# chao1224/GeoSSL

Measured on AMD Instinct MI355X. Metric: molecules/s/GPU SchNet+DDM fwd+bwd (QM9-sized, bs=1024); % HBM roofline, higher is better.
Workload: dtype f32

## Files before the change

geossl_amd/NCSN.py:

```python
import ctypes as C
import os

import numpy as np
import torch
from .switches import env as _env
import torch.nn as nn
import torch.nn.functional as F

from . import _lib
from ._lib import call, ptr, stream
from .layout import get_super_edge_layout


class MultiLayerPerceptron(nn.Module):

    def __init__(self, input_dim, hidden_dims, activation="relu", dropout=0):
        super().__init__()
        self.dims = [input_dim] + hidden_dims
        self.activation = getattr(F, activation) if isinstance(activation, str) else None
        self.dropout = nn.Dropout(dropout) if dropout else None
        self.layers = nn.ModuleList()
        for i in range(len(self.dims) - 1):
            self.layers.append(nn.Linear(self.dims[i], self.dims[i + 1]))
        self.reset_parameters()

    def reset_parameters(self):
        for layer in self.layers:
            nn.init.xavier_uniform_(layer.weight)
            nn.init.constant_(layer.bias, 0.0)

    def forward(self, input):
        from .higher_order import _linear_wide
        _lib.require_cuda(input)
        lead = input.shape[:-1]
        x = input.reshape(-1, input.shape[-1])
        for i, layer in enumerate(self.layers):
            x = _linear_wide(x, layer.weight, layer.bias)
            if i < len(self.layers) - 1:
                if self.activation:
                    x = self.activation(x)
                if self.dropout:
                    x = self.dropout(x)
        return x.reshape(*lead, x.shape[-1])


def _head_params(m):
    i, o = m.input_distance_mlp.layers, m.output_mlp.layers
    return [i[0].weight, i[0].bias, i[1].weight, i[1].bias, o[0].weight, o[0].bias, o[1].weight, o[1].bias,
            o[2].weight, o[2].bias]


_FIELDS = ("in_w1", "in_b1", "in_w2", "in_b2", "o1_w", "o1_b", "o2_w", "o2_b", "o3_w", "o3_b")

_SIDE = {"stream": None, "pending": []}


def set_side_stream(stream):
    _SIDE["stream"] = stream


def join_side_stream():
    if _SIDE["pending"]:
        for ev, _keep in _SIDE["pending"]:
            torch.cuda.current_stream().wait_event(ev)
        _SIDE["pending"].clear()


class _NcsnLoss(torch.autograd.Function):
    @staticmethod
    def forward(ctx, h, distance, noise_level, distance_noise, sel, sigmas, anneal_power, out_scale, *params):
        dev = h.device
        S, Fd = sel.S, h.size(1)
        training = ctx.needs_input_grad[0] or any(ctx.needs_input_grad[8:])
        ps = [p.detach().contiguous() for p in params]
        w = _lib.NcsnWeights()
        for name, p in zip(_FIELDS, ps):
            setattr(w, name, ptr(p))
        w.sigmas = ptr(sigmas)
        ctx.grad_slot = getattr(h, "_geossl_grad_slot", None)
        h = h.detach().contiguous()
        loss_e = torch.empty(S, dtype=torch.float32, device=dev)
        sv = None
        saved = {}
        if training:
            saved = dict(a1=torch.empty(S, Fd, dtype=torch.float32, device=dev),
                         a2=torch.empty(S, Fd // 2, dtype=torch.float32, device=dev),
                         pd=torch.empty(S, dtype=torch.float32, device=dev),
                         emb=torch.empty(S, dtype=torch.float32, device=dev),
                         gscale=torch.empty(S, dtype=torch.float32, device=dev))
            sv = _lib.NcsnSaved(*[ptr(saved[k]) for k in ("a1", "a2", "pd", "emb", "gscale")])
        lib = _lib.load()
        nws = max(int(lib.geossl_ddm_loss_fwd_workspace_floats(Fd)), 256)
        ws = (torch.empty if S > 0 else torch.zeros)(nws, dtype=torch.float32, device=dev)
        st = stream()
        call("geossl_ddm_loss_fwd", ptr(h), ptr(sel.batch), ptr(sel.sei0), ptr(sel.sei1), S,
             ptr(distance.contiguous()), ptr(noise_level.contiguous()), ptr(distance_noise.contiguous()), C.byref(w),
             Fd, float(anneal_power), ptr(loss_e), C.byref(sv) if sv is not None else None, ptr(ws), st)
        loss = torch.empty((), dtype=torch.float32, device=dev)
        call("geossl_loss_reduce_partials", ptr(ws), ptr(sel.stats), float(out_scale), ptr(loss), 0, st)
        if training:
            ctx.sel, ctx.ps, ctx.w, ctx.saved, ctx.h = sel, ps, w, saved, h
            ctx.params = params
            ctx.sigmas = sigmas
            ctx.out_scale = float(out_scale)
        return loss

    @staticmethod
    def backward(ctx, gout):
        sel, ps, w, saved, h = ctx.sel, ctx.ps, ctx.w, ctx.saved, ctx.h
        dev = h.device
        S, Fd, N = sel.S, h.size(1), h.size(0)
        st = stream()
        sv = _lib.NcsnSaved(*[ptr(saved[k]) for k in ("a1", "a2", "pd", "emb", "gscale")])
        dfeat = torch.empty(S, Fd, dtype=torch.float32, device=dev)
        demb = torch.empty(S, dtype=torch.float32, device=dev)
        grow = torch.empty(S, dtype=torch.float32, device=dev)
        gout = gout.contiguous().to(torch.float32)
        direct = _lib.direct_grads_enabled(ctx.params)
        grads = [p.grad for p in ctx.params] if direct else [torch.empty_like(p) for p in ps]
        g = _lib.NcsnGrads(*[ptr(t) for t in grads])
        lib = _lib.load()
        acc = 1 if direct else 0
        split = (_env("GEOSSL_NCSN_SPLIT_BWD") is not None or _env("GEOSSL_ARITH_24BIT") is not None
                 or max(S, N) * Fd * 4 >= 2 ** 32)
        if not split:
            ws1 = torch.empty(int(lib.geossl_ddm_loss_bwd_fused_workspace_floats(S, Fd)), dtype=torch.float32, device=dev)
            call("geossl_ddm_loss_bwd_fused", ptr(h), ptr(sel.sei0), ptr(sel.sei1), S, N, Fd, C.byref(w), C.byref(sv),
                 ptr(sel.stats), ctx.out_scale, ptr(gout), ptr(dfeat), ptr(demb), ptr(grow), C.byref(g), ptr(ws1), acc, st)
            dz1 = None
        else:
            dz1 = torch.empty(S, Fd, dtype=torch.float32, device=dev)
            call("geossl_ddm_loss_bwd_rows", C.byref(w), C.byref(sv), S, Fd, ptr(sel.stats), ctx.out_scale, ptr(gout),
                 ptr(dz1), ptr(dfeat), ptr(demb), ptr(grow), st)
        dh = None
        if ctx.needs_input_grad[0]:
            slot = ctx.grad_slot
            dh = slot.rows(N, Fd, torch.float32, dev) if slot is not None else None
            if dh is None:
                dh = torch.empty(N, Fd, dtype=torch.float32, device=dev)
            call("geossl_incidence_gather", ptr(dfeat), ptr(sel.inc_ptr), ptr(sel.inc_idx), N, Fd, ptr(dh), 0, st)
        if split:
            nfl = lib.geossl_ddm_loss_bwd_workspace_floats(S, Fd)
            side = _SIDE["stream"] if direct else None
            if side is None:
                ws = torch.empty(nfl, dtype=torch.float32, device=dev)
                call("geossl_ddm_loss_bwd_weights", ptr(h), ptr(sel.sei0), ptr(sel.sei1), S, Fd, C.byref(w), C.byref(sv),
                     ptr(dz1), ptr(demb), ptr(grow), C.byref(g), ptr(ws), acc, st)
            else:
                main = torch.cuda.current_stream()
                fork = torch.cuda.Event()
                fork.record(main)
                side.wait_event(fork)
                with torch.cuda.stream(side):
                    ws = torch.empty(nfl, dtype=torch.float32, device=dev)
                    call("geossl_ddm_loss_bwd_weights", ptr(h), ptr(sel.sei0), ptr(sel.sei1), S, Fd, C.byref(w),
                         C.byref(sv), ptr(dz1), ptr(demb), ptr(grow), C.byref(g), ptr(ws), 1, stream())
                    done = torch.cuda.Event()
                    done.record(side)
                _SIDE["pending"].append((done, (h, saved, dz1, demb, grow, ws, w, sv, ps, grads)))
        if direct:
            return (dh, None, None, None, None, None, None, None) + (None,) * len(grads)
        return (dh, None, None, None, None, None, None, None) + tuple(grads)


class _NcsnLossPair(torch.autograd.Function):

    @staticmethod
    def forward(ctx, h1, h2, d1, d2, nl1, dn1, nl2, dn2, sel, sigmas, powers, out_scale, npar, *params):
        dev = h1.device
        S, Fd, N = sel.S, h1.size(1), h1.size(0)
        training = ctx.needs_input_grad[0] or ctx.needs_input_grad[1] or any(ctx.needs_input_grad[13:])
        ps = [p.detach().contiguous() for p in params]
        pss = (ps[:npar], ps[npar:])
        dyn = getattr(sel, "dyn", None)
        ctx.dyn = dyn
        if dyn is not None:
            hs = (h1.detach().contiguous(),) * 2
            ctx.grad_slots = (None, None)
        else:
            hs = (h1.detach().contiguous(), h2.detach().contiguous())
            ctx.grad_slots = (getattr(h1, "_geossl_grad_slot", None), getattr(h2, "_geossl_grad_slot", None))
        heads = (_lib.NcsnHeadFwd * 2)()
        keep, saved, ws = [], [], []
        for k, (h, d, nl, dn) in enumerate(((hs[0], d1, nl1, dn1), (hs[1], d2, nl2, dn2))):
            hd = heads[k]
            d, nl, dn = d.contiguous(), nl.contiguous(), dn.contiguous()
            keep += [d, nl, dn]
            for name, p in zip(_FIELDS, pss[k]):
                setattr(hd.w, name, ptr(p))
            hd.w.sigmas = ptr(sigmas[k])
            hd.h, hd.distance, hd.noise_level, hd.distance_noise = ptr(h), ptr(d), ptr(nl), ptr(dn)
            hd.anneal_power = float(powers[k])
            loss_e = torch.empty(S, dtype=torch.float32, device=dev)
            sv = {}
            if training:
                sv = dict(a1=torch.empty(S, Fd, dtype=torch.float32, device=dev),
                          a2=torch.empty(S, Fd // 2, dtype=torch.float32, device=dev),
                          pd=torch.empty(S, dtype=torch.float32, device=dev),
                          emb=torch.empty(S, dtype=torch.float32, device=dev),
                          gscale=torch.empty(S, dtype=torch.float32, device=dev))
                for name in ("a1", "a2", "pd", "emb", "gscale"):
                    setattr(hd.saved, name, ptr(sv[name]))
            w_ = torch.empty(256, dtype=torch.float32, device=dev)
            hd.loss_e, hd.workspace = ptr(loss_e), ptr(w_)
            keep.append(loss_e)
            saved.append(sv)
            ws.append(w_)
        st = stream()
        call("geossl_ddm_loss_fwd2_dyn", C.byref(heads), ptr(sel.batch), ptr(sel.sei0), ptr(sel.sei1), S, Fd,
             None if dyn is None else dyn.n_super, None if dyn is None else dyn.n_atoms, st)
        loss = torch.empty((), dtype=torch.float32, device=dev)
        call("geossl_loss_reduce_partials2", ptr(ws[0]), ptr(ws[1]), ptr(sel.stats), float(out_scale), float(out_scale),
             ptr(loss), st)
        if training:
            ctx.sel, ctx.pss, ctx.saved, ctx.hs, ctx.sigmas = sel, pss, saved, hs, sigmas
            ctx.params, ctx.npar, ctx.out_scale = params, npar, float(out_scale)
        return loss

    @staticmethod
    def backward(ctx, gout):
        sel, pss, saved, hs = ctx.sel, ctx.pss, ctx.saved, ctx.hs
        dev = hs[0].device
        S, Fd, N = sel.S, hs[0].size(1), hs[0].size(0)
        st = stream()
        gout = gout.contiguous().to(torch.float32)
        direct = _lib.direct_grads_enabled(ctx.params)
        grads = [p.grad for p in ctx.params] if direct else [torch.empty_like(p) for p in pss[0] + pss[1]]
        gs = (grads[:ctx.npar], grads[ctx.npar:])
        lib = _lib.load()
        heads = (_lib.NcsnHeadBwd * 2)()
        keep, dhs = [], []
        nws = int(lib.geossl_ddm_loss_bwd_fused_workspace_floats(S, Fd))
        dyn = ctx.dyn
        dh_all = torch.empty(N, Fd, dtype=torch.float32, device=dev) if dyn is not None else None
        for k in range(2):
            hd = heads[k]
            for name, p in zip(_FIELDS, pss[k]):
                setattr(hd.w, name, ptr(p))
            hd.w.sigmas = ptr(ctx.sigmas[k])
            for name in ("a1", "a2", "pd", "emb", "gscale"):
                setattr(hd.saved, name, ptr(saved[k][name]))
            for name, t_ in zip(_FIELDS, gs[k]):
                setattr(hd.grads, name, ptr(t_))
            dfeat = torch.empty(S, Fd, dtype=torch.float32, device=dev)
            demb = torch.empty(S, dtype=torch.float32, device=dev)
            grow = torch.empty(S, dtype=torch.float32, device=dev)
            ws1 = torch.empty(nws, dtype=torch.float32, device=dev)
            slot = ctx.grad_slots[k]
            dh = dh_all if dyn is not None else (slot.rows(N, Fd, torch.float32, dev) if slot is not None else None)
            if dh is None:
                dh = torch.empty(N, Fd, dtype=torch.float32, device=dev)
            hd.h, hd.out_scale, hd.dfeat, hd.demb, hd.grow, hd.workspace, hd.dh = (
                ptr(hs[k]), ctx.out_scale, ptr(dfeat), ptr(demb), ptr(grow), ptr(ws1), ptr(dh))
            keep += [dfeat, demb, grow, ws1]
            dhs.append(dh)
        call("geossl_ddm_loss_bwd_fused2_dyn", C.byref(heads), ptr(sel.sei0), ptr(sel.sei1), S, sel.N if dyn is not None else N,
             Fd, ptr(sel.stats), ptr(gout), ptr(sel.inc_ptr), ptr(sel.inc_idx), 1 if direct else 0,
             None if dyn is None else dyn.n_super, None if dyn is None else dyn.n_atoms, st)
        head = ((dh_all, None) if dyn is not None else (dhs[0], dhs[1])) + (None,) * 11
        if direct:
            return head + (None,) * len(grads)
        return head + tuple(grads)


def ddm_heads_loss(n1, n2, data, h1, distance_1, h2, distance_2, noise_level_1=None, distance_noise_1=None,
                   noise_level_2=None, distance_noise_2=None, out_scale=0.5):
    ok = (isinstance(n1, NCSN_version_03) and isinstance(n2, NCSN_version_03) and n1.emb_dim == n2.emb_dim
          and n1.emb_dim in (32, 64, 128) and not _env("GEOSSL_NCSN_SPLIT_BWD")
          and not _env("GEOSSL_ARITH_24BIT")
          and not _env("GEOSSL_NCSN_SEPARATE_HEADS")
          and (h2 is None or h1.shape == h2.shape) and not distance_1.requires_grad and not distance_2.requires_grad
          and n1 is not n2 and not ({id(p) for p in _head_params(n1)} & {id(p) for p in _head_params(n2)}))
    if ok:
        S_, N_, Fd = data.super_edge_index.size(1), h1.size(0), h1.size(1)
        ok = S_ > 0 and max(S_, N_) * Fd * 4 < 2 ** 32
    bucket = getattr(data, "_bucket", None)
    if bucket is not None and (not ok or h2 is not None):
        raise _lib.GeosslHipError("a capacity-bucket batch needs the paired NCSN heads on one fused feature tensor")
    if not ok:
        return (n1(data, h1, distance_1, noise_level=noise_level_1, distance_noise=distance_noise_1, out_scale=out_scale) +
                n2(data, h2, distance_2, noise_level=noise_level_2, distance_noise=distance_noise_2, out_scale=out_scale))
    _lib.require_cuda(h1, h2, distance_1, distance_2, n1.sigmas, n2.sigmas)
    n1.device = n2.device = n1.sigmas.device
    num_graphs = data.num_graphs
    sel = bucket.sel if bucket is not None else get_super_edge_layout(data.batch, data.super_edge_index, num_graphs)
    draws = []
    for n_, nl, dn, d in ((n1, noise_level_1, distance_noise_1, distance_1), (n2, noise_level_2, distance_noise_2, distance_2)):
        if nl is None:
            nl = torch.randint(0, n_.sigmas.size(0), (num_graphs,), device=n_.sigmas.device)
        if dn is None:
            dn = torch.randn_like(d)
        draws.append((nl, dn))
    p1, p2 = _head_params(n1), _head_params(n2)
    return _NcsnLossPair.apply(h1, h2, distance_1.view(-1), distance_2.view(-1), draws[0][0], draws[0][1].view(-1),
                               draws[1][0], draws[1][1].view(-1), sel, (n1.sigmas.detach(), n2.sigmas.detach()),
                               (n1.anneal_power, n2.anneal_power), out_scale, len(p1), *p1, *p2)


class NCSN_version_03(torch.nn.Module):
    def __init__(self, emb_dim, sigma_begin, sigma_end, num_noise_level, noise_type, anneal_power):
        super().__init__()
        self.anneal_power = anneal_power
        self.noise_type = noise_type
        self.input_distance_mlp = MultiLayerPerceptron(1, [emb_dim, 1], activation="relu")
        self.output_mlp = MultiLayerPerceptron(1 + emb_dim, [emb_dim, emb_dim // 2, 1])
        sigmas = torch.tensor(np.exp(np.linspace(np.log(sigma_begin), np.log(sigma_end), num_noise_level)),
                              dtype=torch.float32)
        self.sigmas = nn.Parameter(sigmas, requires_grad=False)
        self.emb_dim = emb_dim

    def forward(self, data, node_feature, distance, debug=False, noise_level=None, distance_noise=None,
                out_scale=1.0):
        self.device = self.sigmas.device
        _lib.require_cuda(node_feature, distance, self.sigmas)
        if self.emb_dim not in (32, 64, 128):
            raise NotImplementedError("HIP path supports emb_dim in (32, 64, 128)")
        if distance.requires_grad:
            raise NotImplementedError("gradient w.r.t. distance/positions is not built (SURVEY.md §8(f) N3)")
        num_graphs = data.num_graphs
        sel = get_super_edge_layout(data.batch, data.super_edge_index, num_graphs)
        if noise_level is None:
            noise_level = torch.randint(0, self.sigmas.size(0), (num_graphs,), device=self.device)
        if distance_noise is None:
            distance_noise = torch.randn_like(distance)
        if sel.S == 0:
            raise ValueError("batch has no super edges (scatter_add over an empty index fails in the reference too)")
        loss = _NcsnLoss.apply(node_feature, distance.view(-1), noise_level, distance_noise.view(-1), sel,
                               self.sigmas.detach(), self.anneal_power, out_scale, *_head_params(self))
        if debug:
            print("loss", float(loss))
        return loss
```

geossl_amd/_lib.py:

```python
import ctypes as C
import os

import torch

HERE = os.path.dirname(os.path.abspath(__file__))
LIB_PATH = os.path.join(HERE, "lib", "libgeossl_hip.so")

MAX_L = 12
TN_MAX = 32
EPI_BIAS, EPI_SSP, EPI_RESIDUAL, EPI_MUL_DSSP, CHAIN_SAME_INPUT, CHAIN_NEW_INPUT, CHAIN_ADD_PREV = 1, 2, 4, 8, 16, 32, 64
EPI_SILU, EPI_MUL_DSILU = 128, 256

vp = C.c_void_p
i64 = C.c_int64
i32 = C.c_int
f32 = C.c_float
f64 = C.c_double
u64 = C.c_uint64


class FilterWeights(C.Structure):
    _fields_ = [("w1", vp * MAX_L), ("b1", vp * MAX_L), ("w2", vp * MAX_L), ("b2", vp * MAX_L)]


PREPARE_MAX = 64


class PrepareBatch(C.Structure):
    _fields_ = [("W", vp * PREPARE_MAX), ("image", vp * PREPARE_MAX), ("ldw", i32 * PREPARE_MAX), ("tb", i32 * PREPARE_MAX)]


CHAIN_MAX = 5


class ChainStage(C.Structure):
    _fields_ = [("image", vp), ("bias", vp), ("res", vp), ("tprev", vp), ("out", vp), ("ld", i32), ("flags", i32),
                ("xin", vp), ("ldxin", i32), ("pad_", i32), ("out_act", vp)]


class Chain(C.Structure):
    _fields_ = [("nstage", i32), ("st", ChainStage * CHAIN_MAX)]


LOOP_MAX_OPS = 14


class LoopOp(C.Structure):
    _fields_ = [("kind", i32), ("swap", i32), ("X", vp), ("Wf", vp), ("out", vp), ("chain", Chain)]


class FilterGradIn(C.Structure):
    _fields_ = [("x", vp * MAX_L), ("dagg", vp * MAX_L)]


class FilterGradOut(C.Structure):
    _fields_ = [("dw1", vp * MAX_L), ("db1", vp * MAX_L), ("dw2", vp * MAX_L), ("db2", vp * MAX_L)]


class TnBatch(C.Structure):
    _fields_ = [("A", vp * TN_MAX), ("B", vp * TN_MAX), ("dW", vp * TN_MAX), ("db", vp * TN_MAX)]


class NcsnWeights(C.Structure):
    _fields_ = [(k, vp) for k in ("in_w1", "in_b1", "in_w2", "in_b2", "o1_w", "o1_b", "o2_w", "o2_b", "o3_w", "o3_b",
                                  "sigmas")]


class NcsnGrads(C.Structure):
    _fields_ = [(k, vp) for k in ("in_w1", "in_b1", "in_w2", "in_b2", "o1_w", "o1_b", "o2_w", "o2_b", "o3_w", "o3_b")]


class NcsnSaved(C.Structure):
    _fields_ = [(k, vp) for k in ("a1", "a2", "pd", "emb", "gscale")]


class NcsnHeadFwd(C.Structure):
    _fields_ = [("h", vp), ("distance", vp), ("noise_level", vp), ("distance_noise", vp), ("w", NcsnWeights),
                ("saved", NcsnSaved), ("anneal_power", f32), ("pad_", f32), ("loss_e", vp), ("workspace", vp)]


class NcsnHeadBwd(C.Structure):
    _fields_ = [("h", vp), ("w", NcsnWeights), ("saved", NcsnSaved), ("out_scale", f32), ("pad_", f32), ("dfeat", vp),
                ("demb", vp), ("grow", vp), ("grads", NcsnGrads), ("workspace", vp), ("dh", vp)]


COPY_MAX = 8


class CopyBatch(C.Structure):
    _fields_ = [("dst", vp * COPY_MAX), ("src", vp * COPY_MAX), ("bytes", i64 * COPY_MAX)]


class Gather(C.Structure):
    _fields_ = [(k, vp) for k in ("x_src", "pos_src", "src_off", "mol_ptr", "x_dst", "pos_dst", "batch_dst", "se_ptr", "sei0",
                                  "sei1", "pair_ptr2", "pair_i", "pair_j", "inc_ptr", "inc_idx", "e0_src", "e1_src",
                                  "e_src_off", "e_ptr", "e0_dst", "e1_dst", "zero")] + \
               [("zero_count", i64), ("x_cols", i32), ("option", i32)]


P = C.POINTER
PROTOTYPES = {
    "geossl_abi_version": (i32, []),
    "geossl_layout_build": (i32, [vp, i64, i64, vp, vp, vp, vp]),
    "geossl_pair_index_fill": (i32, [vp, vp, i64, vp, vp, vp]),
    "geossl_radius_graph_count": (i32, [vp, vp, i64, i32, f32, i32, vp, vp]),
    "geossl_radius_graph_fill": (i32, [vp, vp, i64, i32, f32, i32, vp, vp, vp, vp, vp]),
    "geossl_pair_geometry": (i32, [vp, vp, vp, i64, i32, f32, i32, f32, vp, vp, vp, vp]),
    "geossl_rbf_fwd": (i32, [vp, i64, vp, i32, f32, vp, vp]),
    "geossl_ssp_fwd": (i32, [vp, i64, vp, vp]),
    "geossl_ssp_bwd": (i32, [vp, vp, i64, vp, vp]),
    "geossl_cfconv_filter_fwd": (i32, [vp, vp, i64, P(FilterWeights), i32, i32, i32, vp, f32, vp, vp, vp]),
    "geossl_cfconv_filter_bwd_workspace_floats": (i64, [i64, i32, i32, i32]),
    "geossl_cfconv_filter_bwd": (i32, [vp, vp, vp, vp, vp, i64, i64, P(FilterWeights), P(FilterGradIn), i32, i32, i32, vp,
                                       f32, vp, P(FilterGradOut), vp, i32, vp]),
    "geossl_cfconv_filter_dpos": (i32, [vp, vp, vp, vp, vp, i64, P(FilterWeights), P(FilterGradIn), i32, i32, i32, vp, f32,
                                        f32, vp, vp, vp, vp]),
    "geossl_pair_position_grad": (i32, [vp, vp, vp, vp, vp, i64, i64, i32, vp, vp]),
    "geossl_cfconv_aggregate": (i32, [vp, vp, vp, vp, vp, vp, i64, i32, i32, i32, vp, vp]),
    "geossl_aggregate_parts": (i32, [i32]),
    "geossl_cfconv_aggregate_work": (i32, [vp, vp, vp, vp, vp, vp, i64, i32, i32, i32, vp, vp]),
    "geossl_pair_product": (i32, [vp, vp, vp, vp, vp, i64, i32, i32, vp, vp]),
    "geossl_linear": (i32, [vp, i32, vp, vp, vp, vp, vp, i32, i64, i32, i32, i32, i32, vp]),
    "geossl_tn_plan": (None, [i64, i32, P(i32), P(i32)]),
    "geossl_tn_workspace_floats": (i64, [i64, i32, i32, i32]),
    "geossl_row_normalize_fwd": (i32, [vp, i64, i32, f32, vp, vp, vp]),
    "geossl_row_normalize_bwd": (i32, [vp, vp, vp, i64, i32, f32, vp, vp]),
    "geossl_atom_tuples": (i32, [vp, vp, i64, i32, vp, vp, vp]),
    "geossl_linear_image_words": (i64, [i32, i32]),
    "geossl_linear_prepare": (i32, [P(PrepareBatch), i32, i32, i32, i32, vp]),
    "geossl_linear_prepared": (i32, [vp, i32, vp, vp, vp, vp, vp, i32, i64, i32, i32, i32, vp]),
    "geossl_chain_image_words": (i64, [i32]),
    "geossl_chain_prepare": (i32, [P(PrepareBatch), i32, i32, i32, vp]),
    "geossl_linear_chain": (i32, [vp, i32, P(Chain), i64, i32, vp]),
    "geossl_linear_wgrad": (i32, [P(TnBatch), i32, i64, i32, i32, i32, i32, i32, vp, i32, vp]),
    "geossl_embedding_fwd": (i32, [vp, i64, vp, i32, i64, i32, vp, vp, vp]),
    "geossl_embedding_bwd_workspace_floats": (i64, [i32, i32]),
    "geossl_embedding_bwd": (i32, [vp, i64, vp, i32, i64, i32, vp, vp, i32, vp]),
    "geossl_segment_reduce_fwd": (i32, [vp, vp, i64, i32, i32, vp, vp]),
    "geossl_segment_reduce_bwd": (i32, [vp, vp, i64, i32, i32, vp, i32, vp]),
    "geossl_axpy": (i32, [vp, vp, f32, i64, vp, vp]),
    "geossl_pair_distance": (i32, [vp, vp, vp, i64, vp, vp]),
    "geossl_super_edge_ptr": (i32, [vp, vp, vp, i64, i64, vp, vp, vp]),
    "geossl_incidence_count": (i32, [vp, vp, vp, vp, i64, i32, vp, vp]),
    "geossl_incidence_fill": (i32, [vp, vp, vp, vp, i64, i32, vp, vp, vp]),
    "geossl_ddm_loss_fwd_workspace_floats": (i64, [i32]),
    "geossl_ddm_loss_fwd": (i32, [vp, vp, vp, vp, i64, vp, vp, vp, P(NcsnWeights), i32, f32, vp, P(NcsnSaved), vp, vp]),
    "geossl_schnet_layer_loop": (i32, [vp, i32, vp, i32, vp, vp, vp, i32, i32, i64, i32, i32, vp]),
    "geossl_schnet_layer_loop_ragged": (i32, [vp, i32, vp, vp, vp, i64, i32, i64, i32, vp]),
    "geossl_copy2": (i32, [vp, vp, i64, vp, vp, i64, vp]),
    "geossl_ddm_noise": (i32, [vp, f32, f32, i64, i64, i64, i32, i32, vp, vp, vp, vp, vp, vp]),
    "geossl_ddm_noise_seeded": (i32, [u64, f32, f32, i64, i64, i64, i32, i32, vp, vp, vp, vp, vp, vp]),
    "geossl_ddm_views": (i32, [vp, vp, vp, vp, i64, i64, vp, vp, vp, vp, i64, vp, vp]),
    "geossl_loss_reduce_partials": (i32, [vp, vp, f32, vp, i32, vp]),
    "geossl_ddm_loss_fwd2": (i32, [vp, vp, vp, vp, i64, i32, vp]),
    "geossl_loss_reduce_partials2": (i32, [vp, vp, vp, f32, f32, vp, vp]),
    "geossl_ddm_loss_bwd_fused2": (i32, [vp, vp, vp, i64, i64, i32, vp, vp, vp, vp, i32, vp]),
    "geossl_loss_reduce_workspace_floats": (i64, [i64]),
    "geossl_loss_reduce": (i32, [vp, i64, vp, f32, vp, vp, i32, vp]),
    "geossl_ddm_loss_bwd_rows": (i32, [P(NcsnWeights), P(NcsnSaved), i64, i32, vp, f32, vp, vp, vp, vp, vp, vp]),
    "geossl_ddm_loss_bwd_workspace_floats": (i64, [i64, i32]),
    "geossl_ddm_loss_bwd_weights": (i32, [vp, vp, vp, i64, i32, P(NcsnWeights), P(NcsnSaved), vp, vp, vp, P(NcsnGrads),
                                          vp, i32, vp]),
    "geossl_ddm_loss_bwd_fused_workspace_floats": (i64, [i64, i32]),
    "geossl_ddm_loss_bwd_fused": (i32, [vp, vp, vp, i64, i64, i32, P(NcsnWeights), P(NcsnSaved), vp, f32, vp, vp, vp, vp,
                                        P(NcsnGrads), vp, i32, vp]),
    "geossl_incidence_gather": (i32, [vp, vp, vp, i64, i32, vp, i32, vp]),
    "geossl_painn_edge_geom": (i32, [vp, vp, vp, i64, f32, vp, vp, i32, vp, vp, vp, vp]),
    "geossl_silu_fwd": (i32, [vp, i64, vp, vp]),
    "geossl_silu_bwd": (i32, [vp, vp, i64, vp, vp]),
    "geossl_painn_interaction_fwd": (i32, [vp, vp, vp, vp, vp, vp, vp, vp, vp, vp, vp, i64, i32, i32, vp, vp, vp]),
    "geossl_painn_interaction_bwd_workspace_floats": (i64, [i64, i32, i32]),
    "geossl_painn_interaction_fwd_mol": (i32, [vp, vp, vp, vp, vp, vp, vp, vp, vp, vp, vp, vp, i64, i32, i64, i32, i32, vp,
                                               vp, vp]),
    "geossl_painn_interaction_fwd_mma": (i32, [vp, vp, vp, vp, vp, vp, vp, vp, vp, vp, vp, vp, vp, i64, i32, i64, i32, i32,
                                               vp, vp, vp]),
    "geossl_painn_interaction_bwd_mol_workspace_floats": (i64, [i64, i64, i32, i32]),
    "geossl_painn_interaction_bwd_mol": (i32, [vp, vp, vp, vp, vp, vp, vp, vp, vp, vp, vp, vp, vp, i64, i32, i64, i32, i32,
                                               vp, vp, vp, vp, vp, i32, vp]),
    "geossl_painn_interaction_bwd": (i32, [vp, vp, vp, vp, vp, vp, vp, vp, vp, vp, vp, vp, i64, i32, i32, vp, vp, vp, vp,
                                           vp, i32, vp]),
    "geossl_painn_mix_pre_fwd": (i32, [vp, vp, i64, i32, f32, vp, vp, vp]),
    "geossl_painn_mix_post_fwd": (i32, [vp, vp, vp, vp, vp, i64, i32, vp, vp, vp]),
    "geossl_painn_mix_post_bwd": (i32, [vp, vp, vp, vp, vp, i64, i32, vp, vp, vp]),
    "geossl_painn_mix_pre_bwd": (i32, [vp, vp, vp, vp, i64, i32, vp, vp, vp]),
    "geossl_add": (i32, [vp, vp, i64, vp, vp]),
    "geossl_painn_edge_grads": (i32, [vp] * 11 + [i64, i32, i32, vp, vp, vp, i32, vp]),
    "geossl_painn_edge_geom_bwd": (i32, [vp, vp, vp, i64, f32, vp, vp, i32, vp, vp, vp, vp, vp]),
    "geossl_painn_position_grad": (i32, [vp, vp, vp, vp, vp, i64, vp, vp]),
    "geossl_adam_step": (i32, [vp, vp, vp, vp, i64, f64, f64, f64, f64, f64, i64, f32, vp]),
    "geossl_copy_n": (i32, [P(CopyBatch), i32, vp]),
    "geossl_ddm_views_dyn": (i32, [vp, vp, vp, vp, i64, i64, vp, vp, vp, vp, i64, vp, vp, vp, vp]),
    "geossl_embedding_fwd_dyn": (i32, [vp, i64, vp, i32, i64, i32, vp, vp, vp, vp]),
    "geossl_embedding_bwd_dyn": (i32, [vp, i64, vp, i32, i64, i32, vp, vp, i32, vp, vp]),
    "geossl_cfconv_filter_fwd_dyn": (i32, [vp, vp, i64, P(FilterWeights), i32, i32, i32, vp, f32, vp, vp, vp, vp]),
    "geossl_cfconv_filter_bwd_dyn": (i32, [vp, vp, vp, vp, vp, i64, i64, P(FilterWeights), P(FilterGradIn), i32, i32, i32,
                                           vp, f32, vp, P(FilterGradOut), vp, i32, vp, vp, vp]),
    "geossl_cfconv_aggregate_work_dyn": (i32, [vp, vp, vp, vp, vp, vp, i64, i32, i32, i32, vp, vp, vp]),
    "geossl_cfconv_aggregate_targets_dyn": (i32, [vp, vp, vp, vp, vp, vp, i64, i32, i32, i32, vp, vp, vp]),
    "geossl_linear_chain_dyn": (i32, [vp, i32, P(Chain), i64, i32, vp, vp]),
    "geossl_linear_wgrad_dyn": (i32, [P(TnBatch), i32, i64, i32, i32, i32, i32, i32, vp, i32, vp, vp]),
    "geossl_ddm_loss_fwd2_dyn": (i32, [vp, vp, vp, vp, i64, i32, vp, vp, vp]),
    "geossl_ddm_loss_bwd_fused2_dyn": (i32, [vp, vp, vp, i64, i64, i32, vp, vp, vp, vp, i32, vp, vp, vp]),
    "geossl_painn_group_capacity": (i64, [i64, i64]),
    "geossl_painn_edge_layout": (i32, [vp, vp, i64, vp, i64, i64, i64] + [vp] * 12),
    "geossl_painn_edge_geom_dyn": (i32, [vp, vp, vp, i64, f32, vp, vp, i32, vp, vp, vp, vp, vp]),
    "geossl_painn_interaction_fwd_mma_dyn": (i32, [vp, vp, vp, vp, vp, vp, vp, vp, vp, vp, vp, vp, vp, i64, i32, i64, i32,
                                                   i32, vp, vp, vp, vp]),
    "geossl_tape_unary": (i32, [i32, vp, i64, f32, f32, vp, vp]),
    "geossl_tape_binary": (i32, [i32, vp, i32, vp, i32, i64, i32, f32, vp, vp]),
    "geossl_tape_colsum_workspace_floats": (i64, [i64, i32]),
    "geossl_tape_reduce": (i32, [i32, vp, i64, i32, vp, vp, vp]),
    "geossl_tape_gather_rows": (i32, [vp, vp, i32, i64, i32, vp, vp]),
    "geossl_tape_scatter_rows": (i32, [vp, vp, i32, vp, i64, i32, vp, vp]),
    "geossl_tape_copy2d": (i32, [vp, i64, vp, i64, i64, i32, vp]),
    "geossl_tape_fill": (i32, [vp, i64, f32, vp]),
    "geossl_painn_stage_cap": (i32, [i32, i32, i32]),
    "geossl_painn_interaction_fwd_atoms": (i32, [vp] * 12 + [i64, vp, i32, i32, vp, vp, vp]),
    "geossl_painn_interaction_bwd_atoms": (i32, [vp] * 13 + [i64, vp, i32, i32, vp, vp, vp, vp, vp, i32, vp]),
    "geossl_painn_interaction_bwd_mol_skip": (i32, [vp, vp, vp, vp, vp, vp, vp, vp, vp, vp, vp, vp, vp, i64, i32, i64, i32,
                                                    i32, vp, vp, vp, vp, vp, i32, vp]),
    "geossl_painn_mix_pre_fwd_dyn": (i32, [vp, vp, i64, i32, f32, vp, vp, vp, vp]),
    "geossl_painn_mix_post_fwd_dyn": (i32, [vp, vp, vp, vp, vp, i64, i32, vp, vp, vp, vp]),
    "geossl_painn_mix_post_bwd_dyn": (i32, [vp, vp, vp, vp, vp, i64, i32, vp, vp, vp, vp]),
    "geossl_painn_mix_pre_bwd_dyn": (i32, [vp, vp, vp, vp, i64, i32, vp, vp, vp, vp]),
    "geossl_gather_molecules": (i32, [P(Gather), i64, vp]),
}

_lib = None


class GeosslHipError(RuntimeError):
    pass


def load():
    global _lib
    if _lib is not None:
        return _lib
    path = os.environ.get("GEOSSL_HIP_LIB", LIB_PATH)
    if not os.path.exists(path):
        raise GeosslHipError(
            "libgeossl_hip.so is not built (%s). Run `python -m geossl_amd.build` (needs hipcc); "
            "there is no CPU fallback." % path)
    lib = C.CDLL(path)
    for name, (res, args) in PROTOTYPES.items():
        fn = getattr(lib, name)
        fn.restype = res
        fn.argtypes = args
    if lib.geossl_abi_version() != 1:
        raise GeosslHipError("ABI version mismatch")
    _lib = lib
    return lib


def check(rc, what):
    if rc != 0:
        raise GeosslHipError("%s failed with hipError %d" % (what, rc))


def ptr(t):
    if t is None:
        return None
    return t.data_ptr()


def stream():
    return torch._C._cuda_getCurrentRawStream(torch._C._cuda_getDevice())


def require_cuda(*tensors):
    for t in tensors:
        if t is not None and not t.is_cuda:
            raise GeosslHipError(
                "geossl_amd runs on MI355X only: got a %s tensor. The HIP path has no CPU fallback." % t.device.type)



_DIRECT = {"depth": 0}


class direct_grads:
    def __enter__(self):
        _DIRECT["depth"] += 1
        return self

    def __exit__(self, *exc):
        _DIRECT["depth"] -= 1
        return False


def direct_grads_enabled(params):
    return _DIRECT["depth"] > 0 and all(
        p.grad is not None and p.grad.is_contiguous() and p.grad.dtype == torch.float32 and p.grad.is_cuda
        for p in params)


class StatusWord:

    def __init__(self, device, message):
        self.word = torch.zeros(1, dtype=torch.int32, device=device)
        self.host = torch.zeros(1, dtype=torch.int32).pin_memory()
        self.event = None
        self.message = message

    def __deepcopy__(self, memo):
        return None

    def __reduce__(self):
        return (type(None), ())

    def poll(self):
        if self.event is None or torch.cuda.is_current_stream_capturing():
            return
        if self.event.query():
            self.event = None
            if int(self.host[0]):
                raise IndexError(self.message)

    def arm(self, every=1):
        self.calls = getattr(self, "calls", 0) + 1
        if every > 1 and self.calls % every != 1:
            return
        if self.event is None and not torch.cuda.is_current_stream_capturing():
            self.host.copy_(self.word, non_blocking=True)
            self.event = torch.cuda.Event()
            self.event.record()

    def check(self):
        if int(self.word.item()):
            raise IndexError(self.message)


def module_status(module, device, message):
    st = module.__dict__.get("_geossl_status")
    if st is None or st.word.device != device:
        st = StatusWord(device, message)
        module.__dict__["_geossl_status"] = st
    return st


TIMERS = None
CALLS = None


def call(name, *args):
    global CALLS
    lib = load()
    if CALLS is not None:
        CALLS += 1
    timers = TIMERS
    key = name[:-4] if name.endswith("_dyn") else name
    if timers is not None and key in timers:
        e0, e1 = torch.cuda.Event(enable_timing=True), torch.cuda.Event(enable_timing=True)
        e0.record()
        rc = getattr(lib, name)(*args)
        e1.record()
        timers[key].append((e0, e1))
    else:
        rc = getattr(lib, name)(*args)
    check(rc, name)


def fill_ptrs(arr, tensors):
    for i, t in enumerate(tensors):
        arr[i] = ptr(t)
```

geossl_amd/csrc/common.h:

```cpp
#pragma once
#include <hip/hip_runtime.h>
#include <stdint.h>

#include <mutex>

typedef float f32x16 __attribute__((ext_vector_type(16)));
typedef float f32x4 __attribute__((ext_vector_type(4)));

#define GEOSSL_MAX_LAYERS 12
#define GEOSSL_PI_F 3.14159265358979323846f

#define GEOSSL_CHECK_LAUNCH()                  \
  do {                                         \
    hipError_t e__ = hipGetLastError();        \
    if (e__ != hipSuccess) return (int)e__;    \
  } while (0)

namespace geossl {

inline void allow_big_lds_ptr(const void* kernel) {
  struct Seen { const void* fn; int dev; };
  static Seen seen[512];
  static int nseen = 0;
  static std::mutex mu;
  int dev = 0;
  if (hipGetDevice(&dev) != hipSuccess) dev = -1;
  std::lock_guard<std::mutex> lock(mu);
  for (int i = 0; i < nseen; ++i)
    if (seen[i].fn == kernel && seen[i].dev == dev) return;
  (void)hipFuncSetAttribute(kernel, hipFuncAttributeMaxDynamicSharedMemorySize, 160 * 1024);
  if (dev >= 0 && nseen < 512) seen[nseen++] = Seen{kernel, dev};
}
template <typename K>
inline void allow_big_lds(K kernel) { allow_big_lds_ptr(reinterpret_cast<const void*>(kernel)); }


__device__ __forceinline__ float mul_rn(float a, float b) {
#pragma clang fp contract(off)
  return a * b;
}
__device__ __forceinline__ float add_rn(float a, float b) {
#pragma clang fp contract(off)
  return a + b;
}
__device__ __forceinline__ float norm2_rn(float x, float y, float z) {
#pragma clang fp contract(off)
  const float xx = x * x, yy = y * y, zz = z * z;
  return (xx + yy) + zz;
}

__device__ __forceinline__ void lds_barrier() {
  asm volatile("s_waitcnt lgkmcnt(0)\n\ts_barrier" ::: "memory");
}

__device__ __forceinline__ float wave_max(float v) {
  v = fmaxf(v, __builtin_bit_cast(float, __builtin_amdgcn_update_dpp(0, __builtin_bit_cast(int, v), 0xB1, 0xF, 0xF, false)));
  v = fmaxf(v, __builtin_bit_cast(float, __builtin_amdgcn_update_dpp(0, __builtin_bit_cast(int, v), 0x4E, 0xF, 0xF, false)));
  v = fmaxf(v, __builtin_bit_cast(float, __builtin_amdgcn_update_dpp(0, __builtin_bit_cast(int, v), 0x141, 0xF, 0xF, false)));
  v = fmaxf(v, __builtin_bit_cast(float, __builtin_amdgcn_update_dpp(0, __builtin_bit_cast(int, v), 0x140, 0xF, 0xF, false)));
  const float a = __builtin_bit_cast(float, __builtin_amdgcn_readlane(__builtin_bit_cast(int, v), 0));
  const float b = __builtin_bit_cast(float, __builtin_amdgcn_readlane(__builtin_bit_cast(int, v), 16));
  const float c = __builtin_bit_cast(float, __builtin_amdgcn_readlane(__builtin_bit_cast(int, v), 32));
  const float d = __builtin_bit_cast(float, __builtin_amdgcn_readlane(__builtin_bit_cast(int, v), 48));
  return fmaxf(fmaxf(a, b), fmaxf(c, d));
}
__device__ __forceinline__ int wave_max_i32(int v) {
  v = max(v, __builtin_amdgcn_update_dpp(v, v, 0xB1, 0xF, 0xF, false));
  v = max(v, __builtin_amdgcn_update_dpp(v, v, 0x4E, 0xF, 0xF, false));
  v = max(v, __builtin_amdgcn_update_dpp(v, v, 0x141, 0xF, 0xF, false));
  v = max(v, __builtin_amdgcn_update_dpp(v, v, 0x140, 0xF, 0xF, false));
  return max(max(__builtin_amdgcn_readlane(v, 0), __builtin_amdgcn_readlane(v, 16)),
             max(__builtin_amdgcn_readlane(v, 32), __builtin_amdgcn_readlane(v, 48)));
}
__device__ __forceinline__ int c_row(int reg, int lane) { return (reg & 3) + 8 * (reg >> 2) + 4 * (lane >> 5); }

#define GEOSSL_SSP_SHIFT 0.693147182464599609375f
__device__ __forceinline__ float exp_neg(float x) { return __builtin_amdgcn_exp2f(x * 1.44269504088896340736f); }
__device__ __forceinline__ float ssp(float x) {
  const float z = exp_neg(-fabsf(x));
  const float l = __builtin_amdgcn_logf(1.0f + z);
  return fmaf(l, 0.693147180559945309417f, fmaxf(x, 0.0f)) - GEOSSL_SSP_SHIFT;
}
__device__ __forceinline__ float dssp_from_out(float t) { return 1.0f - 0.5f * exp_neg(-t); }

template <class ValFn, class ConsumeFn>
__device__ __forceinline__ void transpose_c_block(float* stage, int lane, ValFn val, ConsumeFn consume) {
  const int j = lane & 31, kh = lane >> 5;
  const int rr = lane >> 3, c4 = lane & 7;
#pragma unroll
  for (int half = 0; half < 2; ++half) {
#pragma unroll
    for (int q = 0; q < 8; ++q) {
      const int r = 8 * half + q;
      const int row16 = (r & 3) + 8 * ((r >> 2) & 1) + 4 * kh;
      stage[row16 * 32 + j] = val(r);
    }
    asm volatile("s_waitcnt lgkmcnt(0)" ::: "memory");
#pragma unroll
    for (int u = 0; u < 2; ++u) {
      const int row16 = 8 * u + rr;
      const float4 v = *reinterpret_cast<const float4*>(stage + row16 * 32 + 4 * c4);
      consume(16 * half + row16, 4 * c4, v);
    }
    asm volatile("s_waitcnt lgkmcnt(0)" ::: "memory");
  }
}

__device__ __forceinline__ float pin(float v) {
  asm volatile("" : "+v"(v));
  return v;
}
__device__ __forceinline__ float4 pin(float4 v) {
  asm volatile("" : "+v"(v.x), "+v"(v.y), "+v"(v.z), "+v"(v.w));
  return v;
}

__device__ __forceinline__ float kahan_sum_strided(const float* __restrict__ p, int b0, int b1, int stride) {
#pragma clang fp reassociate(off) contract(off)
  float s = 0.0f, c = 0.0f;
#pragma unroll 4
  for (int b = b0; b < b1; ++b) {
    const float y = p[(size_t)b * stride] - c;
    const float t = s + y;
    c = (t - s) - y;
    s = t;
  }
  return s;
}

__device__ __forceinline__ int dyn_count(int cap, const int32_t* __restrict__ dyn) {
  return dyn != nullptr ? min(cap, *dyn) : cap;
}

__device__ __forceinline__ float wave_sum(float v) {
#pragma unroll
  for (int o = 32; o > 0; o >>= 1) v += __shfl_xor(v, o, 64);
  return v;
}

}
```

geossl_amd/csrc/ncsn_bwd.hip:

```cpp
#include "common.h"
#include "geossl_hip.h"
#include "split.h"
#include "tn.h"

using namespace geossl;

namespace {

constexpr int TR = 32;

#ifdef NB_TIMING
__device__ long long nb_dbg[2 * 32 * 8];
#define NB_MARK(slot)                                                                              \
  do {                                                                                             \
    if (blockIdx.x == 5 && lane == 0 && (wave == 0 || wave == NW) && t - t_begin < 32)             \
      nb_dbg[((wave == 0 ? 0 : 1) * 32 + (t - t_begin)) * 8 + (slot)] = clock64();                 \
  } while (0)
#else
#define NB_MARK(slot) do {} while (0)
#endif

template <int NW>
struct NbLds {
  static constexpr int F = 32 * NW, H = F / 2, KHS = (H + 15) / 16, HMB = (H + 31) / 32, KS = F / 16;
  u32x4* zb;
  u32x4* dz2T;
  u32x4* fT;
  u32x4* dz1r;
  u32x4* abT;
  int4* scal;
  float* pdv;
  float* dep;
  float* wls;
  int* eg;
  int* ef;
  int* ea;
  int* ec;
  __device__ explicit NbLds(uint8_t* smem) {
    zb = reinterpret_cast<u32x4*>(smem);
    dz2T = zb + 2 * KHS * 2 * 64;
    fT = dz2T + HMB * 2 * 2 * 64;
    dz1r = fT + 2 * NW * 2 * 2 * 64;
    abT = dz1r + KS * 2 * 64;
    scal = reinterpret_cast<int4*>(abT + NW * 2 * 2 * 64);
    pdv = reinterpret_cast<float*>(scal + 3 * TR);
    dep = pdv + 3 * TR;
    wls = dep + NW * TR;
    eg = reinterpret_cast<int*>(wls + F);
    ef = eg + 4;
    ea = ef + 2 * NW;
    ec = ea + NW;
  }
  static size_t bytes() {
    return (size_t)(2 * KHS * 2 + HMB * 4 + 2 * NW * 4 + KS * 2 + NW * 4) * 1024 + 3 * TR * sizeof(int4) +
           (size_t)(3 * TR + NW * TR + F) * sizeof(float) + (size_t)(4 + 4 * NW) * sizeof(int);
  }
};

struct NcsnFusedArgs {
  const float* h;
  const int64_t* sei0;
  const int64_t* sei1;
  int S;
  GeosslNcsnWeights w;
  GeosslNcsnSaved sv;
  const int64_t* divisor;
  float out_scale;
  const float* gout;
  float* dfeat;
  float* demb;
  float* grow;
  float* pw1;
  float* pd1;
  float* pb1;
  float* pw2;
  float* pb2;
  float* psm;
};

__device__ __forceinline__ float ldg_off(const float* base, uint32_t byte_off) {
  return *reinterpret_cast<const float*>(reinterpret_cast<const char*>(base) + byte_off);
}
__device__ __forceinline__ int crow4(int r, int k4) { return (r & 3) + 8 * (r >> 2) + k4; }
__device__ __forceinline__ int opaque(int v) {
  asm volatile("" : "+v"(v));
  return v;
}
__device__ __forceinline__ u32x4 pack8(const f32x16& t, int s) {
  u32x4 w;
#pragma unroll
  for (int q = 0; q < 4; ++q) {
    const f16x2 p = {(_Float16)t[8 * s + 2 * q], (_Float16)t[8 * s + 2 * q + 1]};
    w[q] = __builtin_bit_cast(uint32_t, p);
  }
  return w;
}
__device__ __forceinline__ const u32x4& piece(const Frag2& f, int pc) { return pc == 0 ? f.h : f.l; }
__device__ __forceinline__ int scale_exponent(float m) { return max(mag_exponent(m), -40); }
__device__ __forceinline__ float pow2(int e) { return __builtin_amdgcn_ldexpf(1.0f, e); }
constexpr int E_NONE = -100000;

template <int NW, bool ROLE_A>
__device__ __forceinline__ void ncsn_bwd_body(const NcsnFusedArgs& a, const int S, const float* __restrict__ a_h) {
  using L_t = NbLds<NW>;
  constexpr int F = L_t::F, H = L_t::H, KHS = L_t::KHS, HMB = L_t::HMB, KS = L_t::KS, NT = 128 * NW;
  extern __shared__ __attribute__((aligned(16))) uint8_t smem_raw[];
  const L_t L(smem_raw);
  const int tid = threadIdx.x, lane = tid & 63, j = lane & 31, kh = lane >> 5;
  const int wave = __builtin_amdgcn_readfirstlane(tid >> 6);
  const int nb = ROLE_A ? wave : wave - NW;
  const int ntiles = (S + TR - 1) / TR;
  const int per = (ntiles + (int)gridDim.x - 1) / (int)gridDim.x;
  const int t_begin = (int)blockIdx.x * per, t_end = min(ntiles, t_begin + per);
  const float scale = a.out_scale * (a.gout != nullptr ? a.gout[0] : 1.0f) / (float)a.divisor[0];
  const uint32_t col = 32 * nb + j;

  Frag2 wreg[ROLE_A ? KHS : KS];
  f32x16 accw1[ROLE_A ? NW : 1];
  f32x16 accw2[ROLE_A ? 1 : HMB];
  int E1[ROLE_A ? NW : 1];
  int E2 = E_NONE;
  int ew = 0;
  float bsum = 0.0f, dsum = 0.0f;
  u32x4 ident[2];
  float w3r[8];
  float s_w2 = 0.0f, s_w1 = 0.0f, s_b1 = 0.0f, s_g = 0.0f, s_d = 0.0f;
  float iw1 = 0.0f, ib1 = 0.0f, iw2 = 0.0f;
  int e3;
  {
    float m3 = 0.0f;
    for (int i = lane; i < H; i += 64) m3 = fmaxf(m3, fabsf(a.w.o3_w[i]));
    e3 = scale_exponent(wave_max(m3));
  }
  if constexpr (ROLE_A) {
    iw1 = a.w.in_w1[col];
    ib1 = a.w.in_b1[col];
    iw2 = a.w.in_w2[col];
    float raw[KHS][8];
    float wm = 0.0f, csum = 0.0f;
#pragma unroll
    for (int ks = 0; ks < KHS; ++ks)
#pragma unroll
      for (int e = 0; e < 8; ++e) {
        const int m = 16 * ks + 8 * kh + e;
        const float v = m < H ? a.w.o2_w[(size_t)m * F + col] : 0.0f;
        raw[ks][e] = v;
        wm = fmaxf(wm, fabsf(v));
        csum = fmaf(fabsf(v), m < H ? fabsf(a.w.o3_w[m]) : 0.0f, csum);
      }
    ew = scale_exponent(wave_max(wm));
    const float sw = pow2(14 - ew);
#pragma unroll
    for (int ks = 0; ks < KHS; ++ks) wreg[ks] = split8h_scaled(raw[ks], sw);
    csum += __shfl_xor(csum, 32, 64);
    const int ecw = max(mag_exponent(wave_max(csum)), -80);
    if (lane == 0) L.ec[nb] = ecw;
#pragma unroll
    for (int kb = 0; kb < NW; ++kb) {
      E1[kb] = E_NONE;
#pragma unroll
      for (int r = 0; r < 16; ++r) accw1[kb][r] = 0.0f;
    }
#pragma unroll
    for (int s = 0; s < 2; ++s)
#pragma unroll
      for (int q = 0; q < 4; ++q) {
        const int k0 = 16 * s + kperm(2 * q, kh), k1 = 16 * s + kperm(2 * q + 1, kh);
        ident[s][q] = (k0 == j ? 0x3C00u : 0u) | (k1 == j ? 0x3C000000u : 0u);
      }
  } else {
    float raw[KS][8];
    float wm = 0.0f;
#pragma unroll
    for (int ks = 0; ks < KS; ++ks)
#pragma unroll
      for (int e = 0; e < 8; ++e) {
        raw[ks][e] = a.w.o1_w[(size_t)(16 * ks + kperm(e, kh)) * (F + 1) + col];
        wm = fmaxf(wm, fabsf(raw[ks][e]));
      }
    ew = scale_exponent(wave_max(wm));
    const float sw = pow2(14 - ew);
#pragma unroll
    for (int ks = 0; ks < KS; ++ks) wreg[ks] = split8h_scaled(raw[ks], sw);
#pragma unroll
    for (int e = 0; e < 8; ++e) {
      const int m = 16 * nb + 8 * kh + e;
      w3r[e] = (nb < KHS && m < H) ? a.w.o3_w[m] : 0.0f;
    }
#pragma unroll
    for (int mb = 0; mb < HMB; ++mb)
#pragma unroll
      for (int r = 0; r < 16; ++r) accw2[mb][r] = 0.0f;
#pragma unroll
    for (int q2 = 0; q2 < 2; ++q2)
#pragma unroll
      for (int q = 0; q < 4; ++q) {
        const int k0 = 16 * q2 + 8 * kh + 2 * q;
        ident[q2][q] = (k0 == j ? 0x3C00u : 0u) | (k0 + 1 == j ? 0x3C000000u : 0u);
      }
  }
  for (int i = tid; i < F; i += NT) L.wls[i] = a.w.o1_w[(size_t)i * (F + 1) + F];

  int sc_u = 0, sc_v = 0;
  float sc_g = 0.0f, sc_e = 0.0f, sc_p = 0.0f;
  int EG = -60;
  auto load_scal = [&](int tt) {
    if constexpr (ROLE_A) {
      if (wave == 0) {
        const int row = min(TR * tt + j, S - 1);
        sc_u = (int)a.sei0[row];
        sc_v = (int)a.sei1[row];
        sc_g = a.sv.gscale[row];
        sc_e = a.sv.emb[row];
        sc_p = a.sv.pd[row];
      }
    }
  };
  auto put_scal = [&](int tt) {
    if constexpr (ROLE_A) {
      if (wave == 0) {
        const int row = TR * tt + lane;
        const bool valid = lane < TR && row < S && tt < t_end;
        const float gr = valid ? pin(sc_g) * scale : 0.0f;
        EG = max(EG, mag_exponent(wave_max(fabsf(gr))));
        if (lane < TR) {
          L.scal[(tt % 3) * TR + lane] = make_int4(sc_u, sc_v, __float_as_int(gr), __float_as_int(sc_e));
          L.pdv[(tt % 3) * TR + lane] = sc_p;
          if (valid) a.grow[row] = gr;
        }
        if (lane == 0) L.eg[tt % 3] = EG;
      }
    }
  };
  float a1raw[16];
  auto request_a1 = [&](int tt, int k4) {
    if constexpr (ROLE_A) {
#pragma unroll
      for (int r = 0; r < 16; ++r)
        a1raw[r] = ldg_off(a.sv.a1, ((uint32_t)min(TR * tt + crow4(r, k4), S - 1) * (uint32_t)F + col) * 4u);
    }
  };
  f32x4 a2raw[2];
  float o3acc[8] = {0.0f, 0.0f, 0.0f, 0.0f, 0.0f, 0.0f, 0.0f, 0.0f};
  auto request_a2 = [&](int tt) {
    if constexpr (!ROLE_A) {
      if (nb < KHS) {
        const uint32_t off = ((uint32_t)min(TR * tt + j, S - 1) * (uint32_t)H + (16 * nb + 8 * kh)) * 4u;
        a2raw[0] = *reinterpret_cast<const f32x4*>(reinterpret_cast<const char*>(a.sv.a2) + off);
        a2raw[1] = *reinterpret_cast<const f32x4*>(reinterpret_cast<const char*>(a.sv.a2) + 16 + off);
      }
    }
  };
  float hu[16], hv[16];
  auto request_gather = [&](int tt, int k4) {
    if constexpr (!ROLE_A) {
      const int2* sc = reinterpret_cast<const int2*>(L.scal + (tt % 3) * TR);
#pragma unroll
      for (int r = 0; r < 16; ++r) {
        const int2 uv = sc[2 * crow4(r, k4)];
        hu[r] = ldg_off(a_h, ((uint32_t)uv.x * (uint32_t)F + col) * 4u);
        hv[r] = ldg_off(a_h, ((uint32_t)uv.y * (uint32_t)F + col) * 4u);
      }
    }
  };
  auto build_zb = [&](int tt) {
    if constexpr (!ROLE_A) {
      if (nb < KHS) {
        const float gr = __int_as_float(L.scal[(tt % 3) * TR + j].z);
        const float sz = pow2(14 - e3 - __builtin_amdgcn_readfirstlane(L.eg[tt % 3]));
        const float av[8] = {a2raw[0].x, a2raw[0].y, a2raw[0].z, a2raw[0].w, a2raw[1].x, a2raw[1].y, a2raw[1].z, a2raw[1].w};
        float v[8];
#pragma unroll
        for (int e = 0; e < 8; ++e) {
          const float a2v = pin(av[e]);
          v[e] = a2v > 0.0f ? gr * w3r[e] : 0.0f;
          o3acc[e] = fmaf(gr, a2v, o3acc[e]);
        }
        const Frag2 f = split8h_scaled(v, sz);
        u32x4* dst = L.zb + (size_t)(((tt & 1) * KHS + nb) * 2) * 64 + lane;
        dst[0] = f.h;
        dst[64] = f.l;
      }
    }
  };
  int EF = -40;
  auto build_fT = [&](int tt) {
    if constexpr (!ROLE_A) {
      float v[16];
      float m = 0.0f;
#pragma unroll
      for (int r = 0; r < 16; ++r) {
        v[r] = pin(hu[r]) + pin(hv[r]);
        m = fmaxf(m, fabsf(v[r]));
      }
      EF = max(EF, mag_exponent(wave_max(m)));
      const float sf = pow2(14 - EF);
      if (lane == 0) L.ef[(tt & 1) * NW + nb] = EF;
#pragma unroll
      for (int s = 0; s < 2; ++s) {
        float vv[8];
#pragma unroll
        for (int e = 0; e < 8; ++e) vv[e] = v[8 * s + e];
        const Frag2 f = split8h_scaled(vv, sf);
        u32x4* dst = L.fT + (size_t)((((tt & 1) * NW + nb) * 2 + s) * 2) * 64 + lane;
        dst[0] = f.h;
        dst[64] = f.l;
      }
    }
  };

  load_scal(t_begin);
  put_scal(t_begin);
  load_scal(t_begin + 1);
  put_scal(t_begin + 1);
  load_scal(t_begin + 2);
  if (t_begin < t_end) {
    request_a1(t_begin, 4 * kh);
    request_a2(t_begin);
  }
  __syncthreads();
  int eC = -80;
#pragma unroll
  for (int i = 0; i < NW; ++i) eC = max(eC, __builtin_amdgcn_readfirstlane(L.ec[i]));
  if (t_begin < t_end) {
    request_gather(t_begin, 4 * kh);
    build_zb(t_begin);
    build_fT(t_begin);
    request_a2(t_begin + 1);
    request_gather(t_begin + 1, 4 * kh);
  }
  int EA = -40;
  const float kA = pow2(e3 + ew - eC - 14);
  for (int t = t_begin; t < t_end; ++t) {
    const int buf = t & 1;
    int k4 = opaque(4 * kh);
    NB_MARK(0);
    lds_barrier();
    NB_MARK(1);
    const int EGt = __builtin_amdgcn_readfirstlane(L.eg[t % 3]);
    if constexpr (ROLE_A) {
      put_scal(t + 2);
      const float kT = pow2(EGt + eC - 14);
      f32x16 acc0, acc1;
#pragma unroll
      for (int r = 0; r < 16; ++r) acc0[r] = acc1[r] = 0.0f;
      {
        const u32x4* zs = L.zb + (size_t)(buf * KHS * 2) * 64 + lane;
        Frag2 a0, an;
        a0.h = zs[0]; a0.l = zs[64];
#pragma unroll
        for (int ks = 0; ks < KHS; ++ks) {
          if (ks + 1 < KHS) {
            const u32x4* s0 = zs + (size_t)((ks + 1) * 2) * 64;
            an.h = s0[0]; an.l = s0[64];
          }
          __builtin_amdgcn_sched_barrier(0);
          mma3x2(acc0, acc1, a0, wreg[ks]);
          __builtin_amdgcn_sched_barrier(0);
          if (ks + 1 < KHS) a0 = an;
        }
      }
      NB_MARK(5);
      float v[16];
      {
        const int4* sc = L.scal + (t % 3) * TR;
        float tb = 0.0f, td = 0.0f, am = 0.0f;
#pragma unroll
        for (int r = 0; r < 16; ++r) {
          a1raw[r] = pin(a1raw[r]);
          v[r] = a1raw[r] > 0.0f ? (acc0[r] + acc1[r]) * kA : 0.0f;
          tb += v[r];
          td = fmaf(v[r], __int_as_float(sc[crow4(r, k4)].w), td);
          am = fmaxf(am, fabsf(a1raw[r]));
        }
        bsum = fmaf(tb, kT, bsum);
        dsum = fmaf(td, kT, dsum);
        EA = max(EA, mag_exponent(wave_max(am)));
      }
      {
        const float sa = pow2(14 - EA);
        if (lane == 0) L.ea[nb] = EA;
#pragma unroll
        for (int s = 0; s < 2; ++s) {
          float vv[8];
#pragma unroll
          for (int e = 0; e < 8; ++e) vv[e] = a1raw[8 * s + e];
          const Frag2 f = split8h_scaled(vv, sa);
          u32x4* dst = L.abT + (size_t)((nb * 2 + s) * 2) * 64 + lane;
          dst[0] = f.h;
          dst[64] = f.l;
        }
      }
      Frag2 da[2];
#pragma unroll
      for (int s = 0; s < 2; ++s) {
        float vv[8];
#pragma unroll
        for (int e = 0; e < 8; ++e) vv[e] = v[8 * s + e];
        da[s] = split8h(vv);
      }
      {
        float wl[16];
#pragma unroll
        for (int r = 0; r < 16; ++r) wl[r] = L.wls[32 * nb + crow4(r, k4)];
        float de = 0.0f;
#pragma unroll
        for (int pc = 1; pc >= 0; --pc) {
          f32x16 tp;
#pragma unroll
          for (int r = 0; r < 16; ++r) tp[r] = 0.0f;
          tp = mfma_f16(piece(da[0], pc), ident[0], tp);
          tp = mfma_f16(piece(da[1], pc), ident[1], tp);
#pragma unroll
          for (int r = 0; r < 16; ++r) de = fmaf(tp[r], wl[r], de);
#pragma unroll
          for (int half = 0; half < 2; ++half)
            L.dz1r[(size_t)((2 * nb + half) * 2 + pc) * 64 + lane] = pack8(tp, half);
        }
        de += __shfl_xor(de, 32, 64);
        if (kh == 0) L.dep[j * NW + nb] = de * kT;
      }
      NB_MARK(6);
#pragma unroll
      for (int kb = 0; kb < NW; ++kb) {
        const int En = EGt + __builtin_amdgcn_readfirstlane(L.ef[buf * NW + kb]);
        if (En != E1[kb]) {
          const float f = pow2(max(E1[kb] - En, -200));
#pragma unroll
          for (int r = 0; r < 16; ++r) accw1[kb][r] *= f;
          E1[kb] = En;
        }
#pragma unroll
        for (int s = 0; s < 2; ++s) {
          const u32x4* s0 = L.fT + (size_t)(((buf * NW + kb) * 2 + s) * 2) * 64 + lane;
          Frag2 bf;
          bf.h = s0[0]; bf.l = s0[64];
          mma3(accw1[kb], da[s], bf);
        }
      }
    } else {
      if (nb < HMB) {
        float tb = 0.0f;
#pragma unroll
        for (int pc = 1; pc >= 0; --pc) {
          f32x16 tp;
#pragma unroll
          for (int r = 0; r < 16; ++r) tp[r] = 0.0f;
#pragma unroll
          for (int q = 0; q < 2; ++q) {
            if (2 * nb + q < KHS) {
              const u32x4* s0 = L.zb + (size_t)((buf * KHS + 2 * nb + q) * 2 + pc) * 64 + lane;
              tp = mfma_f16(s0[0], ident[q], tp);
            }
          }
#pragma unroll
          for (int r = 0; r < 16; ++r) tb += tp[r];
#pragma unroll
          for (int s = 0; s < 2; ++s) L.dz2T[(size_t)((nb * 2 + s) * 2 + pc) * 64 + lane] = pack8(tp, s);
        }
        bsum = fmaf(tb, pow2(EGt + e3 - 14), bsum);
      }
      NB_MARK(5);
      build_zb(t + 1);
      NB_MARK(6);
      build_fT(t + 1);
    }
    k4 = opaque(4 * kh);
    NB_MARK(2);
    lds_barrier();
    NB_MARK(3);
    if constexpr (ROLE_A) {
      request_a1(t + 1, k4);
      load_scal(t + 3);
      {
        const int4* sc = L.scal + (t % 3) * TR;
        const float* pdr = L.pdv + (t % 3) * TR;
#pragma unroll
        for (int i = 0; i < 16; ++i) {
          const int rl = 4 * k4 + i;
          float de = 0.0f;
#pragma unroll
          for (int n2 = 0; n2 < NW; ++n2) de += L.dep[rl * NW + n2];
          const float pd = pdr[rl];
          const float pre = fmaf(iw1, pd, ib1);
          s_w2 = fmaf(de, fmaxf(pre, 0.0f), s_w2);
          const float dp = pre > 0.0f ? de * iw2 : 0.0f;
          s_w1 = fmaf(dp, pd, s_w1);
          s_b1 += dp;
          if (wave == 0 && j == i) {
            s_g += __int_as_float(sc[rl].z);
            s_d += de;
          }
        }
      }
    } else {
      request_a2(t + 2);
      request_gather(t + 2, k4);
      NB_MARK(7);
      f32x16 acc0, acc1;
#pragma unroll
      for (int r = 0; r < 16; ++r) acc0[r] = acc1[r] = 0.0f;
      {
        const u32x4* zs = L.dz1r + lane;
        Frag2 b0, bn;
        b0.h = zs[0]; b0.l = zs[64];
#pragma unroll
        for (int ks = 0; ks < KS; ++ks) {
          if (ks + 1 < KS) {
            const u32x4* s0 = zs + (size_t)((ks + 1) * 2) * 64;
            bn.h = s0[0]; bn.l = s0[64];
          }
          __builtin_amdgcn_sched_barrier(0);
          mma3x2(acc0, acc1, wreg[ks], b0);
          __builtin_amdgcn_sched_barrier(0);
          if (ks + 1 < KS) b0 = bn;
        }
      }
      const float kD = pow2(EGt + eC + ew - 28);
      f32x16 outp;
#pragma unroll
      for (int r = 0; r < 16; ++r) outp[r] = (acc0[r] + acc1[r]) * kD;
      const int row = TR * t + j;
      if (row < S) {
        const uint32_t off = ((uint32_t)row * (uint32_t)F + 32 * nb + 4 * kh) * 4u;
#pragma unroll
        for (int q = 0; q < 4; ++q)
          *reinterpret_cast<f32x4*>(reinterpret_cast<char*>(a.dfeat) + 32 * q + off) =
              f32x4{outp[4 * q], outp[4 * q + 1], outp[4 * q + 2], outp[4 * q + 3]};
        if (nb == 0 && kh == 0) {
          float de = 0.0f;
#pragma unroll
          for (int n2 = 0; n2 < NW; ++n2) de += L.dep[j * NW + n2];
          a.demb[row] = de;
        }
      }
      {
        const int En = EGt + __builtin_amdgcn_readfirstlane(L.ea[nb]);
        if (En != E2) {
          const float f = pow2(max(E2 - En, -200));
#pragma unroll
          for (int mb = 0; mb < HMB; ++mb)
#pragma unroll
            for (int r = 0; r < 16; ++r) accw2[mb][r] *= f;
          E2 = En;
        }
      }
#pragma unroll
      for (int s = 0; s < 2; ++s) {
        const u32x4* sb = L.abT + (size_t)((nb * 2 + s) * 2) * 64 + lane;
        Frag2 bf;
        bf.h = sb[0]; bf.l = sb[64];
#pragma unroll
        for (int mb = 0; mb < HMB; ++mb) {
          const u32x4* s0 = L.dz2T + (size_t)((mb * 2 + s) * 2) * 64 + lane;
          Frag2 af;
          af.h = s0[0]; af.l = s0[64];
          mma3(accw2[mb], af, bf);
        }
      }
    }
    NB_MARK(4);
  }
  const size_t pb = blockIdx.x;
  if constexpr (ROLE_A) {
    float* P1 = a.pw1 + pb * F * F;
#pragma unroll
    for (int kb = 0; kb < NW; ++kb) {
      const float f = pow2(max(E1[kb] + eC - 28, -200));
#pragma unroll
      for (int r = 0; r < 16; ++r) P1[(size_t)(32 * nb + c_row(r, lane)) * F + 32 * kb + j] = accw1[kb][r] * f;
    }
    const float sb = bsum + __shfl_xor(bsum, 32, 64), sd = dsum + __shfl_xor(dsum, 32, 64);
    if (kh == 0) {
      a.pb1[pb * F + col] = sb;
      a.pd1[pb * F + col] = sd;
    }
    float* Ps = a.psm + pb * (H + 3 * F + 2);
    const float t_w2 = s_w2 + __shfl_xor(s_w2, 32, 64);
    const float t_w1 = s_w1 + __shfl_xor(s_w1, 32, 64), t_b1 = s_b1 + __shfl_xor(s_b1, 32, 64);
    if (kh == 0) {
      Ps[H + col] = t_w2;
      Ps[H + F + col] = t_w1;
      Ps[H + 2 * F + col] = t_b1;
    }
    if (wave == 0) {
      const float tg = wave_sum(s_g), td = wave_sum(s_d);
      if (lane == 0) {
        Ps[H + 3 * F] = tg;
        Ps[H + 3 * F + 1] = td;
      }
    }
  } else {
    float* P2 = a.pw2 + pb * H * F;
    const float f = pow2(max(E2 + e3 - 28, -200));
#pragma unroll
    for (int mb = 0; mb < HMB; ++mb)
#pragma unroll
      for (int r = 0; r < 16; ++r) {
        const int m = 32 * mb + c_row(r, lane);
        if (m < H) P2[(size_t)m * F + col] = accw2[mb][r] * f;
      }
    const float sb = bsum + __shfl_xor(bsum, 32, 64);
    if (nb < HMB && kh == 0 && (int)col < H) a.pb2[pb * H + col] = sb;
    if (nb < KHS) {
      float* Ps = a.psm + pb * (H + 3 * F + 2);
#pragma unroll
      for (int e = 0; e < 8; ++e) {
        float v = o3acc[e];
#pragma unroll
        for (int o = 16; o > 0; o >>= 1) v += __shfl_xor(v, o, 64);
        const int m = 16 * nb + 8 * kh + e;
        if (j == 0 && m < H) Ps[m] = v;
      }
    }
  }
}

template <int NW>
__global__ __launch_bounds__(128 * NW) void k_ncsn_bwd_fused(NcsnFusedArgs a) {
  if ((int)(threadIdx.x >> 6) < NW) ncsn_bwd_body<NW, true>(a, a.S, a.h);
  else ncsn_bwd_body<NW, false>(a, a.S, a.h);
}
struct NcsnFusedPair { NcsnFusedArgs a[2]; };
template <int NW>
__global__ __launch_bounds__(128 * NW) void k_ncsn_bwd_fused2(NcsnFusedPair pr, const int32_t* __restrict__ dyn_S,
                                                              const int32_t* __restrict__ dyn_view) {
  const NcsnFusedArgs& a = pr.a[blockIdx.y];
  const int S = dyn_count(a.S, dyn_S);
  const float* h = a.h;
  if (dyn_view != nullptr && blockIdx.y == 1) h += (size_t)(*dyn_view) * (32 * NW);
  if ((int)(threadIdx.x >> 6) < NW) ncsn_bwd_body<NW, true>(a, S, h);
  else ncsn_bwd_body<NW, false>(a, S, h);
}

__device__ __forceinline__ void ncsn_reduce_all_block(const ReduceMulti& m, int nblk, int accumulate,
                                                      const float* __restrict__ psm, int F, const GeosslNcsnGrads& g,
                                                      float (*red)[64]) {
  const int mb = m.xoff[m.nseg];
  if ((int)blockIdx.x < mb) {
    reduce_multi_block(m, nblk, accumulate, red, 0);
    return;
  }
  const int H = F / 2, len = H + 3 * F + 2;
  const int i = ((int)blockIdx.x - mb) * 4 + (int)(threadIdx.x >> 6), lane = threadIdx.x & 63;
  if (i >= len) return;
  float s = 0.0f;
  for (int b = lane; b < nblk; b += 64) s += psm[(size_t)b * len + i];
  s = wave_sum(s);
  if (lane == 0) {
    float* dst;
    if (i < H) dst = g.o3_w + i;
    else if (i < H + F) dst = g.in_w2 + (i - H);
    else if (i < H + 2 * F) dst = g.in_w1 + (i - H - F);
    else if (i < H + 3 * F) dst = g.in_b1 + (i - H - 2 * F);
    else if (i == H + 3 * F) dst = g.o3_b;
    else dst = g.in_b2;
    *dst = accumulate ? *dst + s : s;
  }
}
__global__ __launch_bounds__(256) void k_ncsn_reduce_all(ReduceMulti m, int nblk, int accumulate,
                                                         const float* __restrict__ psm, int F, GeosslNcsnGrads g) {
  __shared__ float red[4][64];
  ncsn_reduce_all_block(m, nblk, accumulate, psm, F, g, red);
}
__global__ __launch_bounds__(256) void k_ncsn_reduce_all2(ReduceMulti m0, ReduceMulti m1, int nblk, int accumulate,
                                                          const float* __restrict__ psm0,
                                                          const float* __restrict__ psm1, int F, GeosslNcsnGrads g0,
                                                          GeosslNcsnGrads g1) {
  __shared__ float red[4][64];
  if (blockIdx.y == 0) ncsn_reduce_all_block(m0, nblk, accumulate, psm0, F, g0, red);
  else ncsn_reduce_all_block(m1, nblk, accumulate, psm1, F, g1, red);
}

inline int fused_blocks(int64_t S) {
  const int64_t ntiles = (S + TR - 1) / TR;
  return (int)(ntiles < 256 ? ntiles : 256);
}

}

#ifdef NB_TIMING
extern "C" int geossl_ncsn_bwd_debug_read(long long* host) {
  return (int)hipMemcpyFromSymbol(host, HIP_SYMBOL(nb_dbg), sizeof(long long) * 2 * 32 * 8);
}
#endif

extern "C" int64_t geossl_ddm_loss_bwd_fused_workspace_floats(int64_t S, int F) {
  const int64_t nb = fused_blocks(S), H = F / 2;
  return nb * ((int64_t)F * F + 2 * F + H * F + H + (H + 3 * F + 2));
}

extern "C" int geossl_ddm_loss_bwd_fused(const float* h, const int64_t* sei0, const int64_t* sei1, int64_t S, int64_t N,
                                         int F, const GeosslNcsnWeights* w, const GeosslNcsnSaved* saved,
                                         const int64_t* stats_divisor, float out_scale, const float* gout, float* dfeat,
                                         float* demb, float* grow, const GeosslNcsnGrads* grads, float* workspace,
                                         int accumulate, hipStream_t stream) {
  if (S <= 0) return 0;
  if (F != 32 && F != 64 && F != 128) return (int)hipErrorInvalidValue;
  if (S * (int64_t)F * 4 >= ((int64_t)1 << 32) || N * (int64_t)F * 4 >= ((int64_t)1 << 32)) return (int)hipErrorInvalidValue;
  const int nb = fused_blocks(S), H = F / 2;
  NcsnFusedArgs a;
  a.h = h; a.sei0 = sei0; a.sei1 = sei1; a.S = (int)S; a.w = *w; a.sv = *saved; a.divisor = stats_divisor;
  a.out_scale = out_scale; a.gout = gout; a.dfeat = dfeat; a.demb = demb; a.grow = grow;
  a.pw1 = workspace;
  a.pd1 = a.pw1 + (size_t)nb * F * F;
  a.pb1 = a.pd1 + (size_t)nb * F;
  a.pw2 = a.pb1 + (size_t)nb * F;
  a.pb2 = a.pw2 + (size_t)nb * H * F;
  a.psm = a.pb2 + (size_t)nb * H;
#define LAUNCH(NWV)                                                                                      \
  do {                                                                                                   \
    allow_big_lds(&k_ncsn_bwd_fused<NWV>);                                                               \
    hipLaunchKernelGGL((k_ncsn_bwd_fused<NWV>), dim3(nb), dim3(128 * NWV), NbLds<NWV>::bytes(), stream, a); \
  } while (0)
  if (F == 128) LAUNCH(4); else if (F == 64) LAUNCH(2); else LAUNCH(1);
#undef LAUNCH
  GEOSSL_CHECK_LAUNCH();
  ReduceMulti rm;
  float* o1w[1] = {grads->o1_w};
  float* o1c[1] = {grads->o1_w + F};
  float* o1b[1] = {grads->o1_b};
  float* o2w[1] = {grads->o2_w};
  float* o2b[1] = {grads->o2_b};
  rm.add(a.pw1, F * F, F, F + 1, 1, o1w, 1);
  rm.add(a.pd1, F, F, F, F + 1, o1c, 1);
  rm.add(a.pb1, F, F, F, 1, o1b, 1);
  rm.add(a.pw2, H * F, F, F, 1, o2w, 1);
  rm.add(a.pb2, H, H, H, 1, o2b, 1);
  hipLaunchKernelGGL(k_ncsn_reduce_all, dim3(rm.blocks() + (H + 3 * F + 2 + 3) / 4, 1), dim3(256), 0, stream, rm, nb,
                     accumulate, a.psm, F, *grads);
  GEOSSL_CHECK_LAUNCH();
  return 0;
}

namespace geossl {
int launch_incidence_gather2(const float* dfeat0, const float* dfeat1, const int64_t* inc_ptr, const int32_t* inc_idx,
                             int64_t N, int F, float* dh0, float* dh1, hipStream_t stream, const int32_t* dyn_view);
}

extern "C" int geossl_ddm_loss_bwd_fused2(const GeosslNcsnHeadBwd* heads, const int64_t* sei0, const int64_t* sei1,
                                          int64_t S, int64_t N, int F, const int64_t* stats_divisor, const float* gout,
                                          const int64_t* inc_ptr, const int32_t* inc_idx, int accumulate,
                                          hipStream_t stream) {
  return geossl_ddm_loss_bwd_fused2_dyn(heads, sei0, sei1, S, N, F, stats_divisor, gout, inc_ptr, inc_idx, accumulate,
                                        nullptr, nullptr, stream);
}

extern "C" int geossl_ddm_loss_bwd_fused2_dyn(const GeosslNcsnHeadBwd* heads, const int64_t* sei0, const int64_t* sei1,
                                              int64_t S, int64_t N, int F, const int64_t* stats_divisor,
                                              const float* gout, const int64_t* inc_ptr, const int32_t* inc_idx,
                                              int accumulate, const int32_t* dyn_S, const int32_t* dyn_view,
                                              hipStream_t stream) {
  if (S <= 0) return 0;
  if (heads == nullptr || (F != 32 && F != 64 && F != 128)) return (int)hipErrorInvalidValue;
  if (S * (int64_t)F * 4 >= ((int64_t)1 << 32) || N * (int64_t)F * 4 >= ((int64_t)1 << 32)) return (int)hipErrorInvalidValue;
  const int nb = (fused_blocks(S) + 1) / 2, H = F / 2;
  NcsnFusedPair pr;
  NcsnFusedArgs* a = pr.a;
  for (int k = 0; k < 2; ++k) {
    const GeosslNcsnHeadBwd& hd = heads[k];
    if (hd.h == nullptr || hd.dfeat == nullptr || hd.workspace == nullptr) return (int)hipErrorInvalidValue;
    NcsnFusedArgs& x = a[k];
    x.h = hd.h; x.sei0 = sei0; x.sei1 = sei1; x.S = (int)S; x.w = hd.w; x.sv = hd.saved; x.divisor = stats_divisor;
    x.out_scale = hd.out_scale; x.gout = gout; x.dfeat = hd.dfeat; x.demb = hd.demb; x.grow = hd.grow;
    x.pw1 = hd.workspace;
    x.pd1 = x.pw1 + (size_t)nb * F * F;
    x.pb1 = x.pd1 + (size_t)nb * F;
    x.pw2 = x.pb1 + (size_t)nb * F;
    x.pb2 = x.pw2 + (size_t)nb * H * F;
    x.psm = x.pb2 + (size_t)nb * H;
  }
#define LAUNCH2(NWV)                                                                                                \
  do {                                                                                                              \
    allow_big_lds(&k_ncsn_bwd_fused2<NWV>);                                                                         \
    hipLaunchKernelGGL((k_ncsn_bwd_fused2<NWV>), dim3(nb, 2), dim3(128 * NWV), NbLds<NWV>::bytes(), stream, pr,         \
                       dyn_S, dyn_view);                                                                            \
  } while (0)
  if (F == 128) LAUNCH2(4); else if (F == 64) LAUNCH2(2); else LAUNCH2(1);
#undef LAUNCH2
  GEOSSL_CHECK_LAUNCH();
  ReduceMulti rm[2];
  for (int k = 0; k < 2; ++k) {
    const GeosslNcsnGrads* grads = &heads[k].grads;
    float* o1w[1] = {grads->o1_w};
    float* o1c[1] = {grads->o1_w + F};
    float* o1b[1] = {grads->o1_b};
    float* o2w[1] = {grads->o2_w};
    float* o2b[1] = {grads->o2_b};
    rm[k].add(a[k].pw1, F * F, F, F + 1, 1, o1w, 1);
    rm[k].add(a[k].pd1, F, F, F, F + 1, o1c, 1);
    rm[k].add(a[k].pb1, F, F, F, 1, o1b, 1);
    rm[k].add(a[k].pw2, H * F, F, F, 1, o2w, 1);
    rm[k].add(a[k].pb2, H, H, H, 1, o2b, 1);
  }
  hipLaunchKernelGGL(k_ncsn_reduce_all2, dim3(rm[0].blocks() + (H + 3 * F + 2 + 3) / 4, 2), dim3(256), 0, stream, rm[0],
                     rm[1], nb, accumulate, a[0].psm, a[1].psm, F, heads[0].grads, heads[1].grads);
  GEOSSL_CHECK_LAUNCH();
  if (heads[0].dh != nullptr && heads[1].dh != nullptr)
    return launch_incidence_gather2(heads[0].dfeat, heads[1].dfeat, inc_ptr, inc_idx, N, F, heads[0].dh, heads[1].dh, stream,
                                    dyn_view);
  return 0;
}
```

geossl_amd/csrc/ncsn_rows.hip:

```cpp
#include "common.h"
#include "geossl_hip.h"
#include "split.h"

using namespace geossl;

namespace {

struct RowIn {
  int64_t u, v;
  float sigma, d, eps;
};

template <int NMB>
__device__ __forceinline__ void ncsn_fwd_body(const float* __restrict__ h, const int64_t* __restrict__ batch,
                                              const int64_t* __restrict__ sei0, const int64_t* __restrict__ sei1,
                                              int S, const float* __restrict__ distance,
                                              const int64_t* __restrict__ noise_level,
                                              const float* __restrict__ dist_noise, const GeosslNcsnWeights& w,
                                              float anneal_power, float* __restrict__ loss_e,
                                              const GeosslNcsnSaved& sv, float* __restrict__ loss_part) {
  constexpr int F = 32 * NMB, H = F / 2, HMB = (H + 31) / 32, HP = 32 * HMB, KS = F / 16;
  extern __shared__ __attribute__((aligned(16))) uint8_t smem_raw[];
  u32x4* W1f = reinterpret_cast<u32x4*>(smem_raw);
  u32x4* W2f = W1f + NMB * KS * 3 * 64;
  float* b1s = reinterpret_cast<float*>(W2f + HMB * KS * 3 * 64);
  float* wls = b1s + F;
  float* b2s = wls + F;
  float* w3s = b2s + HP;
  float* iw1 = w3s + HP;
  float* ib1 = iw1 + F;
  float* iw2 = ib1 + F;
  float* lred = iw2 + F;
  const int tid = threadIdx.x, lane = tid & 63, wave = tid >> 6, j = lane & 31, kh = lane >> 5;
  const int nrb = (S + 31) / 32;
  float lsum = 0.0f;
  auto load_row = [&](int rb) {
    RowIn r;
    const int rowc = min(32 * rb + j, S - 1);
    r.u = sei0[rowc];
    r.v = sei1[rowc];
    r.sigma = w.sigmas[noise_level[batch[r.u]]];
    r.d = distance[rowc];
    r.eps = dist_noise[rowc];
    return r;
  };
  int rb = blockIdx.x + gridDim.x * wave;
  RowIn cur;
  if (rb < nrb) cur = load_row(rb);
#ifdef NCSN_STAGE_UNROLL
#pragma unroll
#endif
  for (int i = tid; i < NMB * KS * 64; i += 512) {
    const int ln = i & 63, ks = (i >> 6) % KS, mb = i / (64 * KS);
    const float* row = w.o1_w + (size_t)(32 * mb + (ln & 31)) * (F + 1) + 16 * ks + 8 * (ln >> 5);
    float v[8];
#pragma unroll
    for (int e = 0; e < 8; ++e) v[e] = row[e];
    const Frag3 f = split8(v);
    u32x4* dst = W1f + ((size_t)(mb * KS + ks) * 3) * 64 + ln;
    dst[0] = f.h;
    dst[64] = f.m;
    dst[128] = f.l;
  }
#ifdef NCSN_STAGE_UNROLL
#pragma unroll
#endif
  for (int i = tid; i < HMB * KS * 64; i += 512) {
    const int ln = i & 63, ks = (i >> 6) % KS, mb = i / (64 * KS);
    const int m = 32 * mb + (ln & 31);
    const float* row = w.o2_w + (size_t)min(m, H - 1) * F + 16 * ks + 4 * (ln >> 5);
    const f32x4 lo = *reinterpret_cast<const f32x4*>(row), hi = *reinterpret_cast<const f32x4*>(row + 8);
    float v[8] = {lo.x, lo.y, lo.z, lo.w, hi.x, hi.y, hi.z, hi.w};
    if (m >= H) {
#pragma unroll
      for (int e = 0; e < 8; ++e) v[e] = 0.0f;
    }
    const Frag3 f = split8(v);
    u32x4* dst = W2f + ((size_t)(mb * KS + ks) * 3) * 64 + ln;
    dst[0] = f.h;
    dst[64] = f.m;
    dst[128] = f.l;
  }
  for (int i = tid; i < F; i += 512) {
    b1s[i] = w.o1_b[i];
    wls[i] = w.o1_w[(size_t)i * (F + 1) + F];
    iw1[i] = w.in_w1[i];
    ib1[i] = w.in_b1[i];
    iw2[i] = w.in_w2[i];
  }
  for (int i = tid; i < HP; i += 512) {
    b2s[i] = i < H ? w.o2_b[i] : 0.0f;
    w3s[i] = i < H ? w.o3_w[i] : 0.0f;
  }
  __syncthreads();
  const float ib2 = w.in_b2[0], b3 = w.o3_b[0];
  for (; rb < nrb; rb += gridDim.x * 8) {
    const int row = 32 * rb + j;
    const bool valid = row < S;
    const RowIn in = cur;
    f32x4 gq[2][4];
    auto gather = [&](int ks, f32x4 (&g)[4]) {
      const float* hu = h + (size_t)in.u * F + 16 * ks + 8 * kh;
      const float* hv = h + (size_t)in.v * F + 16 * ks + 8 * kh;
      g[0] = *reinterpret_cast<const f32x4*>(hu);
      g[1] = *reinterpret_cast<const f32x4*>(hu + 4);
      g[2] = *reinterpret_cast<const f32x4*>(hv);
      g[3] = *reinterpret_cast<const f32x4*>(hv + 4);
    };
    gather(0, gq[0]);
    if (rb + gridDim.x * 8 < nrb) cur = load_row(rb + gridDim.x * 8);
    const float pd = add_rn(in.d, mul_rn(in.eps, in.sigma));
    float e = 0.0f;
#pragma unroll 4
    for (int k = kh * (F / 2); k < (kh + 1) * (F / 2); k += 4) {
      const f32x4 a = *reinterpret_cast<const f32x4*>(iw1 + k), b = *reinterpret_cast<const f32x4*>(ib1 + k);
      const f32x4 c = *reinterpret_cast<const f32x4*>(iw2 + k);
      e = fmaf(c.x, fmaxf(fmaf(a.x, pd, b.x), 0.0f), e);
      e = fmaf(c.y, fmaxf(fmaf(a.y, pd, b.y), 0.0f), e);
      e = fmaf(c.z, fmaxf(fmaf(a.z, pd, b.z), 0.0f), e);
      e = fmaf(c.w, fmaxf(fmaf(a.w, pd, b.w), 0.0f), e);
    }
    e += __shfl_xor(e, 32, 64);
    const float emb = e + ib2;
    f32x16 acc1[NMB];
#pragma unroll
    for (int mb = 0; mb < NMB; ++mb)
#pragma unroll
      for (int q = 0; q < 4; ++q) {
        const f32x4 b = *reinterpret_cast<const f32x4*>(b1s + 32 * mb + 8 * q + 4 * kh);
        const f32x4 wl = *reinterpret_cast<const f32x4*>(wls + 32 * mb + 8 * q + 4 * kh);
        acc1[mb][4 * q] = fmaf(emb, wl.x, b.x);
        acc1[mb][4 * q + 1] = fmaf(emb, wl.y, b.y);
        acc1[mb][4 * q + 2] = fmaf(emb, wl.z, b.z);
        acc1[mb][4 * q + 3] = fmaf(emb, wl.w, b.w);
      }
#pragma unroll
    for (int ks = 0; ks < KS; ++ks) {
      if (ks + 1 < KS) gather(ks + 1, gq[(ks + 1) & 1]);
      const f32x4(&g)[4] = gq[ks & 1];
      const float v[8] = {g[0].x + g[2].x, g[0].y + g[2].y, g[0].z + g[2].z, g[0].w + g[2].w,
                          g[1].x + g[3].x, g[1].y + g[3].y, g[1].z + g[3].z, g[1].w + g[3].w};
      const Frag3 bf = split8(v);
      Frag3 af[NMB];
#pragma unroll
      for (int mb = 0; mb < NMB; ++mb) {
        const u32x4* src = W1f + ((size_t)(mb * KS + ks) * 3) * 64 + lane;
        af[mb].h = src[0];
        af[mb].m = src[64];
        af[mb].l = src[128];
      }
#pragma unroll
      for (int mb = 0; mb < NMB; ++mb) acc1[mb] = mfma_bf16(af[mb].l, bf.h, acc1[mb]);
#pragma unroll
      for (int mb = 0; mb < NMB; ++mb) acc1[mb] = mfma_bf16(af[mb].h, bf.l, acc1[mb]);
#pragma unroll
      for (int mb = 0; mb < NMB; ++mb) acc1[mb] = mfma_bf16(af[mb].m, bf.m, acc1[mb]);
#pragma unroll
      for (int mb = 0; mb < NMB; ++mb) acc1[mb] = mfma_bf16(af[mb].m, bf.h, acc1[mb]);
#pragma unroll
      for (int mb = 0; mb < NMB; ++mb) acc1[mb] = mfma_bf16(af[mb].h, bf.m, acc1[mb]);
#pragma unroll
      for (int mb = 0; mb < NMB; ++mb) acc1[mb] = mfma_bf16(af[mb].h, bf.h, acc1[mb]);
      __builtin_amdgcn_sched_barrier(0);
    }
    Frag3 tb[KS];
    {
      float* arow = sv.a1 != nullptr ? sv.a1 + (size_t)row * F + 4 * kh : nullptr;
#pragma unroll
      for (int mb = 0; mb < NMB; ++mb)
#pragma unroll
        for (int half = 0; half < 2; ++half) {
          float v[8];
#pragma unroll
          for (int e2 = 0; e2 < 8; ++e2) v[e2] = fmaxf(acc1[mb][8 * half + e2], 0.0f);
          if (arow != nullptr && valid) {
            *reinterpret_cast<f32x4*>(arow + 32 * mb + 16 * half) = f32x4{v[0], v[1], v[2], v[3]};
            *reinterpret_cast<f32x4*>(arow + 32 * mb + 16 * half + 8) = f32x4{v[4], v[5], v[6], v[7]};
          }
          tb[2 * mb + half] = split8(v);
          __builtin_amdgcn_sched_barrier(0);
        }
    }
    float sc = 0.0f;
#pragma unroll
    for (int mb = 0; mb < HMB; ++mb) {
      f32x16 acc2;
#pragma unroll
      for (int q = 0; q < 4; ++q) {
        const f32x4 b = *reinterpret_cast<const f32x4*>(b2s + 32 * mb + 8 * q + 4 * kh);
        acc2[4 * q] = b.x;
        acc2[4 * q + 1] = b.y;
        acc2[4 * q + 2] = b.z;
        acc2[4 * q + 3] = b.w;
      }
      Frag3 af, an;
      {
        const u32x4* src = W2f + ((size_t)(mb * KS) * 3) * 64 + lane;
        af.h = src[0]; af.m = src[64]; af.l = src[128];
      }
#pragma unroll
      for (int ks = 0; ks < KS; ++ks) {
        if (ks + 1 < KS) {
          const u32x4* src = W2f + ((size_t)(mb * KS + ks + 1) * 3) * 64 + lane;
          an.h = src[0]; an.m = src[64]; an.l = src[128];
        }
        __builtin_amdgcn_sched_barrier(0);
        mma6(acc2, af, tb[ks]);
        __builtin_amdgcn_sched_barrier(0);
        if (ks + 1 < KS) af = an;
      }
      float* a2row = sv.a2 != nullptr ? sv.a2 + (size_t)row * H + 32 * mb + 4 * kh : nullptr;
#pragma unroll
      for (int q = 0; q < 4; ++q) {
        const f32x4 w3 = *reinterpret_cast<const f32x4*>(w3s + 32 * mb + 8 * q + 4 * kh);
        const f32x4 a = f32x4{fmaxf(acc2[4 * q], 0.0f), fmaxf(acc2[4 * q + 1], 0.0f), fmaxf(acc2[4 * q + 2], 0.0f),
                              fmaxf(acc2[4 * q + 3], 0.0f)};
        sc = fmaf(a.x, w3.x, sc);
        sc = fmaf(a.y, w3.y, sc);
        sc = fmaf(a.z, w3.z, sc);
        sc = fmaf(a.w, w3.w, sc);
        if (a2row != nullptr && valid && 32 * mb + 8 * q + 4 * kh < H) *reinterpret_cast<f32x4*>(a2row + 8 * q) = a;
      }
    }
    sc += __shfl_xor(sc, 32, 64);
    const float out = sc + b3;
    const float inv_sigma = 1.0f / in.sigma;
    const float score = out * inv_sigma;
    const float target = (-1.0f / (in.sigma * in.sigma)) * (pd - in.d);
    const float diff = score - target;
    const float pw = powf(in.sigma, anneal_power);
    if (valid && kh == 0) {
      const float le = (0.5f * (diff * diff)) * pw;
      loss_e[row] = le;
      lsum += le;
      if (sv.pd != nullptr) {
        sv.pd[row] = pd;
        sv.emb[row] = emb;
        sv.gscale[row] = diff * pw * inv_sigma;
      }
    }
  }
  if (loss_part != nullptr) {
    lsum = wave_sum(lsum);
    if (lane == 0) lred[wave] = lsum;
    __syncthreads();
    if (tid == 0) {
      float t = 0.0f;
      for (int i = 0; i < 8; ++i) t += lred[i];
      loss_part[blockIdx.x] = t;
    }
    if (blockIdx.x == 0)
      for (int i = (int)gridDim.x + tid; i < GEOSSL_LOSS_PARTIALS; i += 512) loss_part[i] = 0.0f;
  }
}

template <int NMB>
__global__ __launch_bounds__(512) void k_ncsn_fwd(const float* __restrict__ h, const int64_t* __restrict__ batch,
                                                  const int64_t* __restrict__ sei0, const int64_t* __restrict__ sei1,
                                                  int S, const float* __restrict__ distance,
                                                  const int64_t* __restrict__ noise_level,
                                                  const float* __restrict__ dist_noise, GeosslNcsnWeights w,
                                                  float anneal_power, float* __restrict__ loss_e,
                                                  GeosslNcsnSaved sv, float* __restrict__ loss_part) {
  ncsn_fwd_body<NMB>(h, batch, sei0, sei1, S, distance, noise_level, dist_noise, w, anneal_power, loss_e, sv, loss_part);
}
struct NcsnFwdHead {
  const float* h;
  const float* distance;
  const int64_t* noise_level;
  const float* dist_noise;
  GeosslNcsnWeights w;
  GeosslNcsnSaved sv;
  float anneal_power;
  float* loss_e;
  float* loss_part;
};
struct NcsnFwdPair { NcsnFwdHead a[2]; };
template <int NMB>
__global__ __launch_bounds__(512) void k_ncsn_fwd2(NcsnFwdPair pr, const int64_t* __restrict__ batch,
                                                   const int64_t* __restrict__ sei0, const int64_t* __restrict__ sei1,
                                                   int S, const int32_t* __restrict__ dyn_S,
                                                   const int32_t* __restrict__ dyn_view) {
  const NcsnFwdHead& a = pr.a[blockIdx.y];
  const float* h = a.h;
  if (dyn_view != nullptr && blockIdx.y == 1) h += (size_t)(*dyn_view) * (32 * NMB);
  ncsn_fwd_body<NMB>(h, batch, sei0, sei1, dyn_count(S, dyn_S), a.distance, a.noise_level, a.dist_noise, a.w,
                     a.anneal_power, a.loss_e, a.sv, a.loss_part);
}

template <int NMB>
__global__ __launch_bounds__(512) void k_ncsn_bwd_rows(GeosslNcsnWeights w, GeosslNcsnSaved sv, int S,
                                                       const int64_t* __restrict__ divisor, float out_scale,
                                                       const float* __restrict__ gout, float* __restrict__ dz1,
                                                       float* __restrict__ dfeat, float* __restrict__ demb,
                                                       float* __restrict__ grow) {
  constexpr int F = 32 * NMB, H = F / 2, HP = 32 * ((H + 31) / 32), KS = F / 16, KH = H / 16;
  extern __shared__ __attribute__((aligned(16))) uint8_t smem_raw[];
  u32x4* W2t = reinterpret_cast<u32x4*>(smem_raw);
  u32x4* W1t = W2t + NMB * KH * 3 * 64;
  float* wls = reinterpret_cast<float*>(W1t + NMB * KS * 3 * 64);
  float* w3s = wls + F;
  const int tid = threadIdx.x, lane = tid & 63, wave = tid >> 6, j = lane & 31, kh = lane >> 5;
  for (int i = tid; i < NMB * KH * 64; i += 512) {
    const int ln = i & 63, ks = (i >> 6) % KH, mb = i / (64 * KH);
    const float* col = w.o2_w + (size_t)(16 * ks + 8 * (ln >> 5)) * F + 32 * mb + (ln & 31);
    float v[8];
#pragma unroll
    for (int e = 0; e < 8; ++e) v[e] = col[(size_t)e * F];
    const Frag3 f = split8(v);
    u32x4* dst = W2t + ((size_t)(mb * KH + ks) * 3) * 64 + ln;
    dst[0] = f.h;
    dst[64] = f.m;
    dst[128] = f.l;
  }
  for (int i = tid; i < NMB * KS * 64; i += 512) {
    const int ln = i & 63, ks = (i >> 6) % KS, mb = i / (64 * KS);
    const float* col = w.o1_w + 32 * mb + (ln & 31);
    float v[8];
#pragma unroll
    for (int e = 0; e < 8; ++e) v[e] = col[(size_t)(16 * ks + kperm(e, ln >> 5)) * (F + 1)];
    const Frag3 f = split8(v);
    u32x4* dst = W1t + ((size_t)(mb * KS + ks) * 3) * 64 + ln;
    dst[0] = f.h;
    dst[64] = f.m;
    dst[128] = f.l;
  }
  for (int i = tid; i < F; i += 512) wls[i] = w.o1_w[(size_t)i * (F + 1) + F];
  for (int i = tid; i < HP; i += 512) w3s[i] = i < H ? w.o3_w[i] : 0.0f;
  __syncthreads();
  const float scale = out_scale * (gout != nullptr ? gout[0] : 1.0f) / (float)divisor[0];
  const int nrb = (S + 31) / 32;
  for (int rb = blockIdx.x + gridDim.x * wave; rb < nrb; rb += gridDim.x * 8) {
    const int row = 32 * rb + j;
    const bool valid = row < S;
    const size_t rowc = (size_t)min(row, S - 1);
    const float gr = valid ? sv.gscale[rowc] * scale : 0.0f;
    if (valid && kh == 0) grow[row] = gr;
    Frag3 zb[KH];
    {
      const float* a2row = sv.a2 + rowc * H + 8 * kh;
      f32x4 a2v[KH][2];
#pragma unroll
      for (int ks = 0; ks < KH; ++ks) {
        a2v[ks][0] = *reinterpret_cast<const f32x4*>(a2row + 16 * ks);
        a2v[ks][1] = *reinterpret_cast<const f32x4*>(a2row + 16 * ks + 4);
      }
#pragma unroll
      for (int ks = 0; ks < KH; ++ks) {
        const f32x4 w0 = *reinterpret_cast<const f32x4*>(w3s + 16 * ks + 8 * kh);
        const f32x4 w1 = *reinterpret_cast<const f32x4*>(w3s + 16 * ks + 8 * kh + 4);
        const f32x4 a0 = a2v[ks][0], a1 = a2v[ks][1];
        const float v[8] = {a0.x > 0.0f ? gr * w0.x : 0.0f, a0.y > 0.0f ? gr * w0.y : 0.0f,
                            a0.z > 0.0f ? gr * w0.z : 0.0f, a0.w > 0.0f ? gr * w0.w : 0.0f,
                            a1.x > 0.0f ? gr * w1.x : 0.0f, a1.y > 0.0f ? gr * w1.y : 0.0f,
                            a1.z > 0.0f ? gr * w1.z : 0.0f, a1.w > 0.0f ? gr * w1.w : 0.0f};
        zb[ks] = split8(v);
      }
    }
    f32x4 a1v[NMB][4];
    {
      const float* a1row = sv.a1 + rowc * F + 4 * kh;
#pragma unroll
      for (int mb = 0; mb < NMB; ++mb)
#pragma unroll
        for (int q = 0; q < 4; ++q) a1v[mb][q] = *reinterpret_cast<const f32x4*>(a1row + 32 * mb + 8 * q);
    }
    f32x16 acc[NMB];
#pragma unroll
    for (int mb = 0; mb < NMB; ++mb)
#pragma unroll
      for (int r = 0; r < 16; ++r) acc[mb][r] = 0.0f;
#pragma unroll
    for (int ks = 0; ks < KH; ++ks) {
      Frag3 af[NMB];
#pragma unroll
      for (int mb = 0; mb < NMB; ++mb) {
        const u32x4* src = W2t + ((size_t)(mb * KH + ks) * 3) * 64 + lane;
        af[mb].h = src[0];
        af[mb].m = src[64];
        af[mb].l = src[128];
      }
#pragma unroll
      for (int mb = 0; mb < NMB; ++mb) acc[mb] = mfma_bf16(af[mb].l, zb[ks].h, acc[mb]);
#pragma unroll
      for (int mb = 0; mb < NMB; ++mb) acc[mb] = mfma_bf16(af[mb].h, zb[ks].l, acc[mb]);
#pragma unroll
      for (int mb = 0; mb < NMB; ++mb) acc[mb] = mfma_bf16(af[mb].m, zb[ks].m, acc[mb]);
#pragma unroll
      for (int mb = 0; mb < NMB; ++mb) acc[mb] = mfma_bf16(af[mb].m, zb[ks].h, acc[mb]);
#pragma unroll
      for (int mb = 0; mb < NMB; ++mb) acc[mb] = mfma_bf16(af[mb].h, zb[ks].m, acc[mb]);
#pragma unroll
      for (int mb = 0; mb < NMB; ++mb) acc[mb] = mfma_bf16(af[mb].h, zb[ks].h, acc[mb]);
      __builtin_amdgcn_sched_barrier(0);
    }
    Frag3 tb[KS];
    float de = 0.0f;
    {
      float* zrow = dz1 + (size_t)row * F + 4 * kh;
#pragma unroll
      for (int mb = 0; mb < NMB; ++mb)
#pragma unroll
        for (int half = 0; half < 2; ++half) {
          float v[8];
#pragma unroll
          for (int q2 = 0; q2 < 2; ++q2) {
            const f32x4 a = a1v[mb][2 * half + q2];
            const f32x4 wl = *reinterpret_cast<const f32x4*>(wls + 32 * mb + 16 * half + 8 * q2 + 4 * kh);
            v[4 * q2] = a.x > 0.0f ? acc[mb][8 * half + 4 * q2] : 0.0f;
            v[4 * q2 + 1] = a.y > 0.0f ? acc[mb][8 * half + 4 * q2 + 1] : 0.0f;
            v[4 * q2 + 2] = a.z > 0.0f ? acc[mb][8 * half + 4 * q2 + 2] : 0.0f;
            v[4 * q2 + 3] = a.w > 0.0f ? acc[mb][8 * half + 4 * q2 + 3] : 0.0f;
            de = fmaf(v[4 * q2], wl.x, de);
            de = fmaf(v[4 * q2 + 1], wl.y, de);
            de = fmaf(v[4 * q2 + 2], wl.z, de);
            de = fmaf(v[4 * q2 + 3], wl.w, de);
          }
          if (valid) {
            *reinterpret_cast<f32x4*>(zrow + 32 * mb + 16 * half) = f32x4{v[0], v[1], v[2], v[3]};
            *reinterpret_cast<f32x4*>(zrow + 32 * mb + 16 * half + 8) = f32x4{v[4], v[5], v[6], v[7]};
          }
          tb[2 * mb + half] = split8(v);
          __builtin_amdgcn_sched_barrier(0);
        }
    }
    de += __shfl_xor(de, 32, 64);
    if (valid && kh == 0) demb[row] = de;
    float* frow = dfeat + (size_t)row * F + 4 * kh;
    constexpr int MP = NMB >= 2 ? 2 : 1;
#pragma unroll
    for (int mb0 = 0; mb0 < NMB; mb0 += MP) {
      f32x16 acc2[MP];
#pragma unroll
      for (int u = 0; u < MP; ++u)
#pragma unroll
        for (int r = 0; r < 16; ++r) acc2[u][r] = 0.0f;
      Frag3 af[MP], an[MP];
#pragma unroll
      for (int u = 0; u < MP; ++u) {
        const u32x4* src = W1t + ((size_t)((mb0 + u) * KS) * 3) * 64 + lane;
        af[u].h = src[0]; af[u].m = src[64]; af[u].l = src[128];
      }
#pragma unroll
      for (int ks = 0; ks < KS; ++ks) {
        if (ks + 1 < KS) {
#pragma unroll
          for (int u = 0; u < MP; ++u) {
            const u32x4* src = W1t + ((size_t)((mb0 + u) * KS + ks + 1) * 3) * 64 + lane;
            an[u].h = src[0]; an[u].m = src[64]; an[u].l = src[128];
          }
        }
        __builtin_amdgcn_sched_barrier(0);
#pragma unroll
        for (int u = 0; u < MP; ++u) acc2[u] = mfma_bf16(af[u].l, tb[ks].h, acc2[u]);
#pragma unroll
        for (int u = 0; u < MP; ++u) acc2[u] = mfma_bf16(af[u].h, tb[ks].l, acc2[u]);
#pragma unroll
        for (int u = 0; u < MP; ++u) acc2[u] = mfma_bf16(af[u].m, tb[ks].m, acc2[u]);
#pragma unroll
        for (int u = 0; u < MP; ++u) acc2[u] = mfma_bf16(af[u].m, tb[ks].h, acc2[u]);
#pragma unroll
        for (int u = 0; u < MP; ++u) acc2[u] = mfma_bf16(af[u].h, tb[ks].m, acc2[u]);
#pragma unroll
        for (int u = 0; u < MP; ++u) acc2[u] = mfma_bf16(af[u].h, tb[ks].h, acc2[u]);
        __builtin_amdgcn_sched_barrier(0);
        if (ks + 1 < KS) {
#pragma unroll
          for (int u = 0; u < MP; ++u) af[u] = an[u];
        }
      }
      if (valid) {
#pragma unroll
        for (int u = 0; u < MP; ++u)
#pragma unroll
          for (int q = 0; q < 4; ++q)
            *reinterpret_cast<f32x4*>(frow + 32 * (mb0 + u) + 8 * q) =
                f32x4{acc2[u][4 * q], acc2[u][4 * q + 1], acc2[u][4 * q + 2], acc2[u][4 * q + 3]};
      }
    }
  }
}

inline int row_blocks_grid(int64_t S) {
  const int nrb = (int)((S + 31) / 32);
  int nx = (nrb + 7) / 8;
  return nx < 256 ? nx : 256;
}

}

extern "C" int64_t geossl_ddm_loss_fwd_workspace_floats(int F) { return GEOSSL_LOSS_PARTIALS; }

extern "C" int geossl_ddm_loss_fwd(const float* h, const int64_t* batch, const int64_t* sei0, const int64_t* sei1,
                                   int64_t S, const float* distance, const int64_t* noise_level,
                                   const float* distance_noise, const GeosslNcsnWeights* w, int F, float anneal_power,
                                   float* loss_e, const GeosslNcsnSaved* saved, float* workspace, hipStream_t stream) {
  if (S <= 0) return 0;
  if (F != 32 && F != 64 && F != 128) return (int)hipErrorInvalidValue;
  GeosslNcsnSaved sv = {nullptr, nullptr, nullptr, nullptr, nullptr};
  if (saved != nullptr) sv = *saved;
  const int NMB = F / 32, H = F / 2, HMB = (H + 31) / 32, KS = F / 16;
  const size_t lds = (size_t)(NMB + HMB) * KS * 3 * 1024 + (size_t)(5 * F + 2 * 32 * HMB + 8) * sizeof(float);
  dim3 grid(row_blocks_grid(S));
#define LAUNCH(NMBV)                                                                                              \
  do {                                                                                                            \
    allow_big_lds(&k_ncsn_fwd<NMBV>);                                                                             \
    hipLaunchKernelGGL((k_ncsn_fwd<NMBV>), grid, dim3(512), lds, stream, h, batch, sei0, sei1, (int)S, distance,  \
                       noise_level, distance_noise, *w, anneal_power, loss_e, sv, workspace);                     \
  } while (0)
  if (F == 128) LAUNCH(4); else if (F == 64) LAUNCH(2); else LAUNCH(1);
#undef LAUNCH
  GEOSSL_CHECK_LAUNCH();
  return 0;
}

extern "C" int geossl_ddm_loss_fwd2(const GeosslNcsnHeadFwd* heads, const int64_t* batch, const int64_t* sei0,
                                    const int64_t* sei1, int64_t S, int F, hipStream_t stream) {
  return geossl_ddm_loss_fwd2_dyn(heads, batch, sei0, sei1, S, F, nullptr, nullptr, stream);
}

extern "C" int geossl_ddm_loss_fwd2_dyn(const GeosslNcsnHeadFwd* heads, const int64_t* batch, const int64_t* sei0,
                                        const int64_t* sei1, int64_t S, int F, const int32_t* dyn_S,
                                        const int32_t* dyn_view, hipStream_t stream) {
  if (S <= 0) return 0;
  if (heads == nullptr || (F != 32 && F != 64 && F != 128)) return (int)hipErrorInvalidValue;
  NcsnFwdPair pr;
  NcsnFwdHead* a = pr.a;
  for (int k = 0; k < 2; ++k) {
    const GeosslNcsnHeadFwd& hd = heads[k];
    if (hd.h == nullptr || hd.loss_e == nullptr) return (int)hipErrorInvalidValue;
    a[k].h = hd.h; a[k].distance = hd.distance; a[k].noise_level = hd.noise_level; a[k].dist_noise = hd.distance_noise;
    a[k].w = hd.w; a[k].sv = hd.saved; a[k].anneal_power = hd.anneal_power; a[k].loss_e = hd.loss_e;
    a[k].loss_part = hd.workspace;
  }
  const int NMB = F / 32, H = F / 2, HMB = (H + 31) / 32, KS = F / 16;
  const size_t lds = (size_t)(NMB + HMB) * KS * 3 * 1024 + (size_t)(5 * F + 2 * 32 * HMB + 8) * sizeof(float);
  dim3 grid((row_blocks_grid(S) + 1) / 2, 2);
#define LAUNCH(NMBV)                                                                                              \
  do {                                                                                                            \
    allow_big_lds(&k_ncsn_fwd2<NMBV>);                                                                            \
    hipLaunchKernelGGL((k_ncsn_fwd2<NMBV>), grid, dim3(512), lds, stream, pr, batch, sei0, sei1, (int)S,           \
                       dyn_S, dyn_view);                                                                          \
  } while (0)
  if (F == 128) LAUNCH(4); else if (F == 64) LAUNCH(2); else LAUNCH(1);
#undef LAUNCH
  GEOSSL_CHECK_LAUNCH();
  return 0;
}

extern "C" int geossl_ddm_loss_bwd_rows(const GeosslNcsnWeights* w, const GeosslNcsnSaved* saved, int64_t S, int F,
                                        const int64_t* stats_divisor, float out_scale, const float* gout, float* dz1,
                                        float* dfeat, float* demb, float* grow, hipStream_t stream) {
  if (S <= 0) return 0;
  if (F != 32 && F != 64 && F != 128) return (int)hipErrorInvalidValue;
  const int NMB = F / 32, H = F / 2, KS = F / 16, KH = H / 16;
  const size_t lds = (size_t)NMB * (KS + KH) * 3 * 1024 + (size_t)(F + 32 * ((H + 31) / 32)) * sizeof(float);
  dim3 grid(row_blocks_grid(S));
#define LAUNCH(NMBV)                                                                                              \
  do {                                                                                                            \
    allow_big_lds(&k_ncsn_bwd_rows<NMBV>);                                                                        \
    hipLaunchKernelGGL((k_ncsn_bwd_rows<NMBV>), grid, dim3(512), lds, stream, *w, *saved, (int)S, stats_divisor,  \
                       out_scale, gout, dz1, dfeat, demb, grow);                                                  \
  } while (0)
  if (F == 128) LAUNCH(4); else if (F == 64) LAUNCH(2); else LAUNCH(1);
#undef LAUNCH
  GEOSSL_CHECK_LAUNCH();
  return 0;
}
```

include/geossl_hip.h:

```cpp
#ifndef GEOSSL_HIP_H
#define GEOSSL_HIP_H
#include <stdint.h>
#ifdef __HIPCC__
#include <hip/hip_runtime.h>
#else
typedef struct ihipStream_t* hipStream_t;
#endif

#ifdef __cplusplus
extern "C" {
#endif

#define GEOSSL_ABI_VERSION 1
#define GEOSSL_MAX_L 12
#define GEOSSL_TN_MAX 32
#define GEOSSL_LOSS_PARTIALS 256

#define GEOSSL_EPI_BIAS 1
#define GEOSSL_EPI_SSP 2
#define GEOSSL_EPI_RESIDUAL 4
#define GEOSSL_EPI_MUL_DSSP 8
#define GEOSSL_CHAIN_NEW_INPUT 32
#define GEOSSL_CHAIN_ADD_PREV 64
#define GEOSSL_EPI_SILU 128
#define GEOSSL_EPI_MUL_DSILU 256
#define GEOSSL_CHAIN_SAME_INPUT 16

int geossl_abi_version(void);

int geossl_layout_build(const int64_t* batch, int64_t N, int64_t B, int32_t* mol_ptr, int32_t* pair_ptr,
                        int64_t* stats, hipStream_t stream);
int geossl_atom_tuples(const int32_t* mol_ptr, const int64_t* tuple_ptr, int64_t B, int option, int64_t* out0,
                       int64_t* out1, hipStream_t stream);
int geossl_pair_index_fill(const int32_t* mol_ptr, const int32_t* pair_ptr, int64_t B, int32_t* pair_i,
                           int32_t* pair_j, hipStream_t stream);

int geossl_radius_graph_count(const float* pos, const int32_t* mol_ptr, int64_t B, int max_n, float r2, int cap,
                              int32_t* deg, hipStream_t stream);
int geossl_radius_graph_fill(const float* pos, const int32_t* mol_ptr, int64_t B, int max_n, float r2, int cap,
                             const int64_t* edge_ptr, int64_t* edge_src, int64_t* edge_dst, float* edge_weight,
                             hipStream_t stream);
int geossl_pair_geometry(const float* pos, const int32_t* mol_ptr, const int32_t* pair_ptr, int64_t B, int max_n,
                         float r2, int cap, float cutoff, float* pair_d, float* pair_c, uint8_t* pair_flag,
                         hipStream_t stream);

int geossl_rbf_fwd(const float* d, int64_t E, const float* offset, int G, float coeff, float* out,
                   hipStream_t stream);

int geossl_ssp_fwd(const float* x, int64_t n, float* y, hipStream_t stream);
int geossl_ssp_bwd(const float* y, const float* dy, int64_t n, float* dx, hipStream_t stream);

typedef struct {
  const float* w1[GEOSSL_MAX_L];
  const float* b1[GEOSSL_MAX_L];
  const float* w2[GEOSSL_MAX_L];
  const float* b2[GEOSSL_MAX_L];
} GeosslFilterWeights;
int geossl_cfconv_filter_fwd(const float* pair_d, const float* pair_c, int64_t P, const GeosslFilterWeights* w, int L,
                             int F, int G, const float* offset, float coeff, float* T, float* Wf, hipStream_t stream);

typedef struct {
  const float* x[GEOSSL_MAX_L];
  const float* dagg[GEOSSL_MAX_L];
} GeosslFilterGradIn;
typedef struct {
  float* dw1[GEOSSL_MAX_L];
  float* db1[GEOSSL_MAX_L];
  float* dw2[GEOSSL_MAX_L];
  float* db2[GEOSSL_MAX_L];
} GeosslFilterGradOut;
int64_t geossl_cfconv_filter_bwd_workspace_floats(int64_t P, int L, int F, int G);
int geossl_cfconv_filter_bwd(const float* pair_d, const float* pair_c, const uint8_t* pair_flag, const int32_t* pair_i,
                             const int32_t* pair_j, int64_t P, int64_t N, const GeosslFilterWeights* w,
                             const GeosslFilterGradIn* g, int L, int F, int G, const float* offset, float coeff,
                             const float* T, const GeosslFilterGradOut* out, float* workspace, int accumulate,
                             hipStream_t stream);

int geossl_cfconv_filter_dpos(const float* pair_d, const float* pair_c, const uint8_t* pair_flag, const int32_t* pair_i,
                              const int32_t* pair_j, int64_t P, const GeosslFilterWeights* w,
                              const GeosslFilterGradIn* g, int L, int F, int G, const float* offset, float coeff,
                              float cutoff, const float* T, const float* Wf, float* dd, hipStream_t stream);
int geossl_pair_position_grad(const float* pos, const float* pair_d, const float* dd, const int32_t* mol_ptr,
                              const int32_t* pair_ptr, int64_t B, int64_t P, int L, float* dpos, hipStream_t stream);

int geossl_cfconv_aggregate(const float* x, const float* Wf, const uint8_t* pair_flag, const int32_t* mol_ptr,
                            const int32_t* pair_ptr, const int32_t* order, int64_t B, int max_n, int F, int swap,
                            float* out, hipStream_t stream);
int geossl_aggregate_parts(int n);
int geossl_cfconv_aggregate_targets_dyn(const float* x, const float* Wf, const uint8_t* pair_flag, const int32_t* mol_ptr,
                                        const int32_t* pair_ptr, const int32_t* work, int64_t nwork, int max_n, int F,
                                        int swap, float* out, const int32_t* dyn_nwork, hipStream_t stream);
int geossl_cfconv_aggregate_work(const float* x, const float* Wf, const uint8_t* pair_flag, const int32_t* mol_ptr,
                                 const int32_t* pair_ptr, const int32_t* work, int64_t nwork, int max_n, int F,
                                 int swap, float* out, hipStream_t stream);

int geossl_pair_product(const float* a, const float* b, const int32_t* pair_i, const int32_t* pair_j,
                        const uint8_t* pair_flag, int64_t P, int F, int swap, float* out, hipStream_t stream);

int geossl_linear(const float* X, int ldx, const float* W, const float* bias, const float* res, const float* tprev,
                  float* Y, int ldy, int64_t R, int K, int NO, int transB, int flags, hipStream_t stream);

#define GEOSSL_PREPARE_MAX 64
typedef struct {
  const float* W[GEOSSL_PREPARE_MAX];
  uint32_t* image[GEOSSL_PREPARE_MAX];
  int ldw[GEOSSL_PREPARE_MAX];
  int tb[GEOSSL_PREPARE_MAX];
} GeosslPrepareBatch;
int64_t geossl_linear_image_words(int K, int NO);
int geossl_linear_prepare(const GeosslPrepareBatch* batch, int nprob, int K, int NO, int transB, hipStream_t stream);
int geossl_linear_prepared(const float* X, int ldx, const uint32_t* image, const float* bias, const float* res,
                           const float* tprev, float* Y, int ldy, int64_t R, int K, int NO, int flags,
                           hipStream_t stream);

#define GEOSSL_CHAIN_MAX 5
typedef struct {
  const uint32_t* image;
  const float* bias;
  const float* res;
  const float* tprev;
  float* out;
  int ld;
  int flags;
  const float* xin;
  int ldxin;
  int pad_;
  float* out_act;
} GeosslChainStage;
typedef struct {
  int nstage;
  GeosslChainStage st[GEOSSL_CHAIN_MAX];
} GeosslChain;
int64_t geossl_chain_image_words(int F);
int geossl_chain_prepare(const GeosslPrepareBatch* batch, int nprob, int F, int transB, hipStream_t stream);
int geossl_linear_chain(const float* X, int ldx, const GeosslChain* chain, int64_t R, int F, hipStream_t stream);

#define GEOSSL_LOOP_MAX_OPS 14
typedef struct {
  int kind;
  int swap;
  const float* X;
  const float* Wf;
  float* out;
  GeosslChain chain;
} GeosslLoopOp;
int geossl_schnet_layer_loop(const GeosslLoopOp* ops, int nops, const int32_t* plan, int nblocks, const int32_t* mol_ptr,
                             const int32_t* pair_ptr, const uint8_t* pair_flag, int max_n, int uniform, int64_t N, int F,
                             int stagger, hipStream_t stream);
int geossl_schnet_layer_loop_ragged(const GeosslLoopOp* ops, int nops, const int32_t* mol_ptr, const int32_t* pair_ptr,
                                    const uint8_t* pair_flag, int64_t B, int mols_per_block, int64_t N, int F,
                                    hipStream_t stream);

typedef struct {
  const float* A[GEOSSL_TN_MAX];
  const float* B[GEOSSL_TN_MAX];
  float* dW[GEOSSL_TN_MAX];
  float* db[GEOSSL_TN_MAX];
} GeosslTnBatch;
typedef struct {
  float* out[GEOSSL_TN_MAX];
} GeosslReduceBatch;
void geossl_tn_plan(int64_t R, int nprob, int* chunk, int* nblk);
int64_t geossl_tn_workspace_floats(int64_t R, int M, int N, int nprob);
int geossl_linear_wgrad(const GeosslTnBatch* batch, int nprob, int64_t R, int M, int N, int lda, int ldb, int ldw,
                        float* workspace, int accumulate, hipStream_t stream);

int geossl_embedding_fwd(const int64_t* z, int64_t z_stride, const float* table, int num_classes, int64_t N, int F,
                         float* out, int32_t* status, hipStream_t stream);
int64_t geossl_embedding_bwd_workspace_floats(int num_classes, int F);
int geossl_embedding_bwd(const int64_t* z, int64_t z_stride, const float* dh, int num_classes, int64_t N, int F,
                         float* dtable, float* workspace, int accumulate, hipStream_t stream);

int geossl_segment_reduce_fwd(const float* h, const int32_t* mol_ptr, int64_t B, int F, int mean, float* out,
                              hipStream_t stream);
int geossl_row_normalize_fwd(const float* h, int64_t N, int F, float eps, float* y, float* norm, hipStream_t stream);
int geossl_row_normalize_bwd(const float* g, const float* y, const float* norm, int64_t N, int F, float eps,
                             float* dh, hipStream_t stream);
int geossl_segment_reduce_bwd(const float* dout, const int32_t* mol_ptr, int64_t B, int F, int mean, float* dh,
                              int accumulate, hipStream_t stream);

int geossl_axpy(const float* a, const float* b, float alpha, int64_t n, float* out, hipStream_t stream);
int geossl_pair_distance(const float* pos, const int64_t* sei0, const int64_t* sei1, int64_t S, float* out,
                         hipStream_t stream);
int geossl_copy2(void* dst0, const void* src0, int64_t bytes0, void* dst1, const void* src1, int64_t bytes1,
                 hipStream_t stream);
int geossl_ddm_noise(const int64_t* seed, float mu, float sigma, int64_t n_pos, int64_t S, int64_t B, int K1, int K2,
                     float* pos_noise, int64_t* noise_level_1, float* distance_noise_1, int64_t* noise_level_2,
                     float* distance_noise_2, hipStream_t stream);
int geossl_ddm_noise_seeded(uint64_t seed, float mu, float sigma, int64_t n_pos, int64_t S, int64_t B, int K1, int K2,
                            float* pos_noise, int64_t* noise_level_1, float* distance_noise_1, int64_t* noise_level_2,
                            float* distance_noise_2, hipStream_t stream);
int geossl_ddm_views(const float* pos, const float* noise, const int64_t* sei0, const int64_t* sei1, int64_t N, int64_t S,
                     float* pos2, float* d01, float* d02, const int64_t* z, int64_t z_stride, int64_t* z2,
                     hipStream_t stream);
int geossl_super_edge_ptr(const int64_t* batch, const int64_t* sei0, const int64_t* sei1, int64_t S, int64_t B,
                          int32_t* se_ptr, int64_t* stats, hipStream_t stream);
int geossl_incidence_count(const int64_t* batch, const int64_t* sei0, const int64_t* sei1, const int32_t* se_ptr,
                           int64_t N, int sides, int32_t* inc_cnt, hipStream_t stream);
int geossl_incidence_fill(const int64_t* batch, const int64_t* sei0, const int64_t* sei1, const int32_t* se_ptr,
                          int64_t N, int sides, const int64_t* inc_ptr, int32_t* inc_idx, hipStream_t stream);

typedef struct {
  const float* in_w1;
  const float* in_b1;
  const float* in_w2;
  const float* in_b2;
  const float* o1_w;
  const float* o1_b;
  const float* o2_w;
  const float* o2_b;
  const float* o3_w;
  const float* o3_b;
  const float* sigmas;
} GeosslNcsnWeights;
typedef struct {
  float* in_w1; float* in_b1; float* in_w2; float* in_b2;
  float* o1_w; float* o1_b; float* o2_w; float* o2_b; float* o3_w; float* o3_b;
} GeosslNcsnGrads;
typedef struct {
  float* a1; float* a2; float* pd; float* emb; float* gscale;
} GeosslNcsnSaved;
int64_t geossl_ddm_loss_fwd_workspace_floats(int F);
int geossl_ddm_loss_fwd(const float* h, const int64_t* batch, const int64_t* sei0, const int64_t* sei1, int64_t S,
                        const float* distance, const int64_t* noise_level, const float* distance_noise,
                        const GeosslNcsnWeights* w, int F, float anneal_power, float* loss_e,
                        const GeosslNcsnSaved* saved, float* workspace, hipStream_t stream);
int64_t geossl_loss_reduce_workspace_floats(int64_t S);
int geossl_loss_reduce(const float* loss_e, int64_t S, const int64_t* stats_divisor, float out_scale, float* loss,
                       float* workspace, int accumulate, hipStream_t stream);
typedef struct {
  const float* h;
  const float* distance;
  const int64_t* noise_level;
  const float* distance_noise;
  GeosslNcsnWeights w;
  GeosslNcsnSaved saved;
  float anneal_power;
  float pad_;
  float* loss_e;
  float* workspace;
} GeosslNcsnHeadFwd;
typedef struct {
  const float* h;
  GeosslNcsnWeights w;
  GeosslNcsnSaved saved;
  float out_scale;
  float pad_;
  float* dfeat;
  float* demb;
  float* grow;
  GeosslNcsnGrads grads;
  float* workspace;
  float* dh;
} GeosslNcsnHeadBwd;
int geossl_ddm_loss_fwd2(const GeosslNcsnHeadFwd* heads, const int64_t* batch, const int64_t* sei0, const int64_t* sei1,
                         int64_t S, int F, hipStream_t stream);
int geossl_loss_reduce_partials2(const float* partial0, const float* partial1, const int64_t* stats_divisor, float scale0,
                                 float scale1, float* loss, hipStream_t stream);
int geossl_ddm_loss_bwd_fused2(const GeosslNcsnHeadBwd* heads, const int64_t* sei0, const int64_t* sei1, int64_t S,
                               int64_t N, int F, const int64_t* stats_divisor, const float* gout, const int64_t* inc_ptr,
                               const int32_t* inc_idx, int accumulate, hipStream_t stream);
int geossl_loss_reduce_partials(const float* partial, const int64_t* stats_divisor, float out_scale, float* loss,
                                int accumulate, hipStream_t stream);
int geossl_ddm_loss_bwd_rows(const GeosslNcsnWeights* w, const GeosslNcsnSaved* saved, int64_t S, int F,
                             const int64_t* stats_divisor, float out_scale, const float* gout, float* dz1,
                             float* dfeat, float* demb, float* grow, hipStream_t stream);
int64_t geossl_ddm_loss_bwd_workspace_floats(int64_t S, int F);
int geossl_ddm_loss_bwd_weights(const float* h, const int64_t* sei0, const int64_t* sei1, int64_t S, int F,
                                const GeosslNcsnWeights* w, const GeosslNcsnSaved* saved, const float* dz1,
                                const float* demb, const float* grow, const GeosslNcsnGrads* grads,
                                float* workspace, int accumulate, hipStream_t stream);
int64_t geossl_ddm_loss_bwd_fused_workspace_floats(int64_t S, int F);
int geossl_ddm_loss_bwd_fused(const float* h, const int64_t* sei0, const int64_t* sei1, int64_t S, int64_t N, int F,
                              const GeosslNcsnWeights* w, const GeosslNcsnSaved* saved, const int64_t* stats_divisor,
                              float out_scale, const float* gout, float* dfeat, float* demb, float* grow,
                              const GeosslNcsnGrads* grads, float* workspace, int accumulate, hipStream_t stream);
int geossl_incidence_gather(const float* dfeat, const int64_t* inc_ptr, const int32_t* inc_idx, int64_t N, int F,
                            float* dh, int accumulate, hipStream_t stream);

int geossl_painn_edge_geom(const float* pos, const int64_t* idx_i, const int64_t* idx_j, int64_t E, float cutoff,
                           const float* offsets, const float* widths, int R, float* dir, float* fcut, float* phi,
                           hipStream_t stream);
int geossl_silu_fwd(const float* u, int64_t n, float* y, hipStream_t stream);
int geossl_silu_bwd(const float* u, const float* dy, int64_t n, float* du, hipStream_t stream);
int geossl_painn_interaction_fwd(const float* q, const float* mu, const float* xc, const int64_t* idx_j,
                                 const int64_t* inc_ptr, const int32_t* inc_idx, const float* phi, const float* fcut,
                                 const float* dir, const float* Wf, const float* bf, int64_t N, int F, int R,
                                 float* q_out, float* mu_out, hipStream_t stream);
int64_t geossl_painn_interaction_bwd_workspace_floats(int64_t N, int F, int R);
int geossl_painn_interaction_bwd(const float* dq_out, const float* dmu_out, const float* mu, const float* xc,
                                 const int64_t* idx_i, const int64_t* inc_ptr, const int32_t* inc_idx, const float* phi,
                                 const float* fcut, const float* dir, const float* Wf, const float* bf, int64_t N, int F,
                                 int R, float* dxc, float* dmu_in, float* dWf, float* dbf, float* workspace,
                                 int accumulate, hipStream_t stream);
int geossl_painn_interaction_fwd_mma(const float* q, const float* mu, const float* xc, const int64_t* idx_j,
                                     const int32_t* row_edge, const int32_t* grp_atom, const int32_t* mol_grp,
                                     const float* phi, const float* fcut, const float* dir, const float* Wf,
                                     const float* bf, const int32_t* mol_ptr, int64_t B, int max_n, int64_t N, int F, int R,
                                     float* q_out, float* mu_out, hipStream_t stream);
int geossl_painn_interaction_fwd_mol(const float* q, const float* mu, const float* xc, const int64_t* idx_j,
                                     const int64_t* inc_ptr, const int32_t* inc_idx, const float* phi, const float* fcut,
                                     const float* dir, const float* Wf, const float* bf, const int32_t* mol_ptr,
                                     int64_t B, int max_n, int64_t N, int F, int R, float* q_out, float* mu_out,
                                     hipStream_t stream);
int64_t geossl_painn_interaction_bwd_mol_workspace_floats(int64_t N, int64_t B, int F, int R);
int geossl_painn_interaction_bwd_mol(const float* dq_out, const float* dmu_out, const float* mu, const float* xc,
                                     const int64_t* idx_i, const int64_t* inc_ptr, const int32_t* inc_idx,
                                     const float* phi, const float* fcut, const float* dir, const float* Wf,
                                     const float* bf, const int32_t* mol_ptr, int64_t B, int max_n, int64_t N, int F,
                                     int R, float* dxc, float* dmu_in, float* dWf, float* dbf, float* workspace,
                                     int accumulate, hipStream_t stream);
int geossl_painn_mix_pre_fwd(const float* q, const float* mm, int64_t N, int F, float eps, float* ctx, float* dot,
                             hipStream_t stream);
int geossl_painn_mix_post_fwd(const float* q, const float* mu, const float* mm, const float* xx, const float* dot,
                              int64_t N, int F, float* q_out, float* mu_out, hipStream_t stream);
int geossl_painn_mix_post_bwd(const float* dq_new, const float* dmu_new, const float* mm, const float* xx,
                              const float* dot, int64_t N, int F, float* dxx, float* dmm, hipStream_t stream);
int geossl_painn_mix_pre_bwd(const float* dq_new, const float* dctx, const float* ctx, const float* mm, int64_t N, int F,
                             float* dq_in, float* dmm, hipStream_t stream);
int geossl_add(const float* a, const float* b, int64_t n, float* out, hipStream_t stream);

int geossl_painn_edge_grads(const float* dq_out, const float* dmu_out, const float* mu, const float* xc,
                            const int64_t* idx_i, const int64_t* idx_j, const float* phi, const float* fcut,
                            const float* dir, const float* Wf, const float* bf, int64_t E, int F, int R, float* dphi,
                            float* dfcut, float* ddir, int accumulate, hipStream_t stream);
int geossl_painn_edge_geom_bwd(const float* pos, const int64_t* idx_i, const int64_t* idx_j, int64_t E, float cutoff,
                               const float* offsets, const float* widths, int R, const float* dphi, const float* dfcut,
                               const float* ddir, float* dr, hipStream_t stream);
int geossl_painn_position_grad(const float* dr, const int64_t* inc_i_ptr, const int32_t* inc_i_idx,
                               const int64_t* inc_j_ptr, const int32_t* inc_j_idx, int64_t N, float* dpos,
                               hipStream_t stream);

int geossl_adam_step(float* param, const float* grad, float* exp_avg, float* exp_avg_sq, int64_t n, double lr,
                     double beta1, double beta2, double eps, double weight_decay, int64_t step_count, float grad_scale,
                     hipStream_t stream);

#define GEOSSL_COPY_MAX 8
typedef struct GeosslCopyBatch {
  void* dst[GEOSSL_COPY_MAX];
  const void* src[GEOSSL_COPY_MAX];
  int64_t bytes[GEOSSL_COPY_MAX];
} GeosslCopyBatch;
int geossl_copy_n(const GeosslCopyBatch* batch, int n, hipStream_t stream);
int geossl_ddm_views_dyn(const float* pos, const float* noise, const int64_t* sei0, const int64_t* sei1, int64_t N,
                         int64_t S, float* pos2, float* d01, float* d02, const int64_t* z, int64_t z_stride, int64_t* z2,
                         const int32_t* dyn_N, const int32_t* dyn_S, hipStream_t stream);
int geossl_embedding_fwd_dyn(const int64_t* z, int64_t z_stride, const float* table, int num_classes, int64_t N, int F,
                             float* out, int32_t* status, const int32_t* dyn_N, hipStream_t stream);
int geossl_embedding_bwd_dyn(const int64_t* z, int64_t z_stride, const float* dh, int num_classes, int64_t N, int F,
                             float* dtable, float* workspace, int accumulate, const int32_t* dyn_N, hipStream_t stream);
int geossl_cfconv_filter_fwd_dyn(const float* pair_d, const float* pair_c, int64_t P, const GeosslFilterWeights* w, int L,
                                 int F, int G, const float* offset, float coeff, float* T, float* Wf,
                                 const int32_t* dyn_P, hipStream_t stream);
int geossl_cfconv_filter_bwd_dyn(const float* pair_d, const float* pair_c, const uint8_t* pair_flag,
                                 const int32_t* pair_i, const int32_t* pair_j, int64_t P, int64_t N,
                                 const GeosslFilterWeights* w, const GeosslFilterGradIn* g, int L, int F, int G,
                                 const float* offset, float coeff, const float* T, const GeosslFilterGradOut* out,
                                 float* workspace, int accumulate, const int32_t* dyn_P, const int32_t* dyn_N,
                                 hipStream_t stream);
int geossl_cfconv_aggregate_work_dyn(const float* x, const float* Wf, const uint8_t* pair_flag, const int32_t* mol_ptr,
                                     const int32_t* pair_ptr, const int32_t* work, int64_t nwork, int max_n, int F,
                                     int swap, float* out, const int32_t* dyn_nwork, hipStream_t stream);
int geossl_linear_chain_dyn(const float* X, int ldx, const GeosslChain* chain, int64_t R, int F, const int32_t* dyn_R,
                            hipStream_t stream);
int geossl_linear_wgrad_dyn(const GeosslTnBatch* batch, int nprob, int64_t R, int M, int N, int lda, int ldb, int ldw,
                            float* workspace, int accumulate, const int32_t* dyn_R, hipStream_t stream);
int geossl_ddm_loss_fwd2_dyn(const GeosslNcsnHeadFwd* heads, const int64_t* batch, const int64_t* sei0,
                             const int64_t* sei1, int64_t S, int F, const int32_t* dyn_S, const int32_t* dyn_view,
                             hipStream_t stream);
int geossl_ddm_loss_bwd_fused2_dyn(const GeosslNcsnHeadBwd* heads, const int64_t* sei0, const int64_t* sei1, int64_t S,
                                   int64_t N, int F, const int64_t* stats_divisor, const float* gout,
                                   const int64_t* inc_ptr, const int32_t* inc_idx, int accumulate, const int32_t* dyn_S,
                                   const int32_t* dyn_view, hipStream_t stream);

int64_t geossl_painn_group_capacity(int64_t E2, int64_t N2);
int geossl_painn_edge_layout(const int64_t* src_i, const int64_t* src_j, int64_t E, const int32_t* mol_ptr, int64_t N,
                             int64_t B, int64_t N2cap, int64_t* idx_i2, int64_t* idx_j2, int64_t* iptr_i,
                             int32_t* ilist_i, int64_t* iptr_j, int32_t* ilist_j, int32_t* row_edge, int32_t* grp_atom,
                             int32_t* mol_grp, int32_t* mol_grp_end, int32_t* status, hipStream_t stream);
int geossl_painn_edge_geom_dyn(const float* pos, const int64_t* idx_i, const int64_t* idx_j, int64_t E, float cutoff,
                               const float* offsets, const float* widths, int R, float* dir, float* fcut, float* phi,
                               const int32_t* dyn_E, hipStream_t stream);
int geossl_painn_interaction_fwd_mma_dyn(const float* q, const float* mu, const float* xc, const int64_t* idx_j,
                                         const int32_t* row_edge, const int32_t* grp_atom, const int32_t* mol_grp,
                                         const float* phi, const float* fcut, const float* dir, const float* Wf,
                                         const float* bf, const int32_t* mol_ptr, int64_t B, int max_n, int64_t N, int F,
                                         int R, float* q_out, float* mu_out, const int32_t* mol_grp_end,
                                         hipStream_t stream);
int geossl_painn_stage_cap(int kind, int F, int R);
int geossl_painn_interaction_fwd_atoms(const float* q, const float* mu, const float* xc, const int64_t* idx_j,
                                       const int64_t* inc_ptr, const int32_t* inc_idx, const float* phi,
                                       const float* fcut, const float* dir, const float* Wf, const float* bf,
                                       const int32_t* atom_list, int64_t nlist, const int32_t* dyn_nlist, int F, int R,
                                       float* q_out, float* mu_out, hipStream_t stream);
int geossl_painn_interaction_bwd_atoms(const float* dq_out, const float* dmu_out, const float* mu, const float* xc,
                                       const int64_t* idx_i, const int64_t* inc_ptr, const int32_t* inc_idx,
                                       const float* phi, const float* fcut, const float* dir, const float* Wf,
                                       const float* bf, const int32_t* atom_list, int64_t nlist,
                                       const int32_t* dyn_nlist, int F, int R, float* dxc, float* dmu_in, float* dWf,
                                       float* dbf, float* workspace, int accumulate, hipStream_t stream);
int geossl_painn_interaction_bwd_mol_skip(const float* dq_out, const float* dmu_out, const float* mu, const float* xc,
                                          const int64_t* idx_i, const int64_t* inc_ptr, const int32_t* inc_idx,
                                          const float* phi, const float* fcut, const float* dir, const float* Wf,
                                          const float* bf, const int32_t* mol_ptr, int64_t B, int max_n, int64_t N, int F,
                                          int R, float* dxc, float* dmu_in, float* dWf, float* dbf, float* workspace,
                                          int accumulate, hipStream_t stream);
int geossl_painn_mix_pre_fwd_dyn(const float* q, const float* mm, int64_t N, int F, float eps, float* ctx, float* dot,
                                 const int32_t* dyn_N, hipStream_t stream);
int geossl_painn_mix_post_fwd_dyn(const float* q, const float* mu, const float* mm, const float* xx, const float* dot,
                                  int64_t N, int F, float* q_out, float* mu_out, const int32_t* dyn_N,
                                  hipStream_t stream);
int geossl_painn_mix_post_bwd_dyn(const float* dq_new, const float* dmu_new, const float* mm, const float* xx,
                                  const float* dot, int64_t N, int F, float* dxx, float* dmm, const int32_t* dyn_N,
                                  hipStream_t stream);
int geossl_painn_mix_pre_bwd_dyn(const float* dq_new, const float* dctx, const float* ctx, const float* mm, int64_t N,
                                 int F, float* dq_in, float* dmm, const int32_t* dyn_N, hipStream_t stream);

int geossl_tape_unary(int kind, const float* x, int64_t n, float alpha, float beta, float* y, hipStream_t stream);
int geossl_tape_binary(int op, const float* a, int amode, const float* b, int bmode, int64_t R, int D, float scale,
                       float* y, hipStream_t stream);
int64_t geossl_tape_colsum_workspace_floats(int64_t R, int D);
int geossl_tape_reduce(int kind, const float* x, int64_t R, int D, float* y, float* workspace, hipStream_t stream);
int geossl_tape_gather_rows(const float* src, const void* idx, int idx64, int64_t E, int D, float* out,
                            hipStream_t stream);
int geossl_tape_scatter_rows(const float* src, const void* ptr, int ptr64, const int32_t* perm, int64_t N, int D,
                             float* out, hipStream_t stream);
int geossl_tape_copy2d(const float* src, int64_t ld_src, float* dst, int64_t ld_dst, int64_t R, int C,
                       hipStream_t stream);
int geossl_tape_fill(float* dst, int64_t n, float value, hipStream_t stream);

typedef struct GeosslGather {
  const int64_t* x_src;
  const float* pos_src;
  const int32_t* src_off;
  const int32_t* mol_ptr;
  int64_t* x_dst;
  float* pos_dst;
  int64_t* batch_dst;
  const int32_t* se_ptr;
  int64_t* sei0;
  int64_t* sei1;
  const int32_t* pair_ptr2;
  int32_t* pair_i;
  int32_t* pair_j;
  const int64_t* inc_ptr;
  int32_t* inc_idx;
  const int64_t* e0_src;
  const int64_t* e1_src;
  const int32_t* e_src_off;
  const int32_t* e_ptr;
  int64_t* e0_dst;
  int64_t* e1_dst;
  float* zero;
  int64_t zero_count;
  int32_t x_cols;
  int32_t option;
} GeosslGather;
int geossl_gather_molecules(const GeosslGather* g, int64_t B, hipStream_t stream);

#ifdef __cplusplus
}
#endif
#endif
```

Measured before the change: 394,500.

## Precompute per-atom first-layer projection and gather it per super-edge in NCSN head

The first MLP layer of the DDM/NCSN head is linear in the concatenated pair features, so it is now computed once per atom (N×F projection) in a new MFMA kernel. The forward and backward kernels then gather the two endpoint projections per super-edge and add the distance-embedding term instead of doing a per-edge GEMM. The backward pass also recomputes a1 from the projection rather than reading a saved S×F a1 buffer. This cuts redundant matmul work and memory traffic when S is much larger than N, at the cost of an extra kernel launch, an N×F buffer and gathered (non-coalesced) loads.

```diff
diff --git a/geossl_amd/NCSN.py b/geossl_amd/NCSN.py
--- a/geossl_amd/NCSN.py
+++ b/geossl_amd/NCSN.py
@@ -93,7 +93,8 @@
         nws = max(int(lib.geossl_ddm_loss_fwd_workspace_floats(Fd)), 256)
         ws = (torch.empty if S > 0 else torch.zeros)(nws, dtype=torch.float32, device=dev)
         st = stream()
-        call("geossl_ddm_loss_fwd", ptr(h), ptr(sel.batch), ptr(sel.sei0), ptr(sel.sei1), S,
+        proj = torch.empty(max(h.size(0), 1), Fd, dtype=torch.float32, device=dev)
+        call("geossl_ddm_loss_fwd_proj", ptr(h), h.size(0), ptr(proj), ptr(sel.batch), ptr(sel.sei0), ptr(sel.sei1), S,
              ptr(distance.contiguous()), ptr(noise_level.contiguous()), ptr(distance_noise.contiguous()), C.byref(w),
              Fd, float(anneal_power), ptr(loss_e), C.byref(sv) if sv is not None else None, ptr(ws), st)
         loss = torch.empty((), dtype=torch.float32, device=dev)
@@ -193,17 +194,17 @@
             hd.anneal_power = float(powers[k])
             loss_e = torch.empty(S, dtype=torch.float32, device=dev)
             sv = {}
+            proj = torch.empty(max(N, 1), Fd, dtype=torch.float32, device=dev)
             if training:
-                sv = dict(a1=torch.empty(S, Fd, dtype=torch.float32, device=dev),
-                          a2=torch.empty(S, Fd // 2, dtype=torch.float32, device=dev),
+                sv = dict(a2=torch.empty(S, Fd // 2, dtype=torch.float32, device=dev),
                           pd=torch.empty(S, dtype=torch.float32, device=dev),
                           emb=torch.empty(S, dtype=torch.float32, device=dev),
-                          gscale=torch.empty(S, dtype=torch.float32, device=dev))
-                for name in ("a1", "a2", "pd", "emb", "gscale"):
+                          gscale=torch.empty(S, dtype=torch.float32, device=dev), proj=proj)
+                for name in ("a2", "pd", "emb", "gscale"):
                     setattr(hd.saved, name, ptr(sv[name]))
             w_ = torch.empty(256, dtype=torch.float32, device=dev)
-            hd.loss_e, hd.workspace = ptr(loss_e), ptr(w_)
-            keep.append(loss_e)
+            hd.loss_e, hd.workspace, hd.proj, hd.n_atoms = ptr(loss_e), ptr(w_), ptr(proj), N
+            keep += [loss_e, proj]
             saved.append(sv)
             ws.append(w_)
         st = stream()
@@ -238,8 +239,9 @@
             for name, p in zip(_FIELDS, pss[k]):
                 setattr(hd.w, name, ptr(p))
             hd.w.sigmas = ptr(ctx.sigmas[k])
-            for name in ("a1", "a2", "pd", "emb", "gscale"):
+            for name in ("a2", "pd", "emb", "gscale"):
                 setattr(hd.saved, name, ptr(saved[k][name]))
+            hd.proj = ptr(saved[k]["proj"])
             for name, t_ in zip(_FIELDS, gs[k]):
                 setattr(hd.grads, name, ptr(t_))
             dfeat = torch.empty(S, Fd, dtype=torch.float32, device=dev)
diff --git a/geossl_amd/_lib.py b/geossl_amd/_lib.py
--- a/geossl_amd/_lib.py
+++ b/geossl_amd/_lib.py
@@ -76,12 +76,14 @@
 
 class NcsnHeadFwd(C.Structure):
     _fields_ = [("h", vp), ("distance", vp), ("noise_level", vp), ("distance_noise", vp), ("w", NcsnWeights),
-                ("saved", NcsnSaved), ("anneal_power", f32), ("pad_", f32), ("loss_e", vp), ("workspace", vp)]
+                ("saved", NcsnSaved), ("anneal_power", f32), ("pad_", f32), ("loss_e", vp), ("workspace", vp),
+                ("proj", vp), ("n_atoms", i64)]
 
 
 class NcsnHeadBwd(C.Structure):
     _fields_ = [("h", vp), ("w", NcsnWeights), ("saved", NcsnSaved), ("out_scale", f32), ("pad_", f32), ("dfeat", vp),
-                ("demb", vp), ("grow", vp), ("grads", NcsnGrads), ("workspace", vp), ("dh", vp)]
+                ("demb", vp), ("grow", vp), ("grads", NcsnGrads), ("workspace", vp), ("dh", vp),
+                ("proj", vp)]
 
 
 COPY_MAX = 8
@@ -145,6 +147,8 @@
     "geossl_incidence_fill": (i32, [vp, vp, vp, vp, i64, i32, vp, vp, vp]),
     "geossl_ddm_loss_fwd_workspace_floats": (i64, [i32]),
     "geossl_ddm_loss_fwd": (i32, [vp, vp, vp, vp, i64, vp, vp, vp, P(NcsnWeights), i32, f32, vp, P(NcsnSaved), vp, vp]),
+    "geossl_ddm_loss_fwd_proj": (i32, [vp, i64, vp, vp, vp, vp, i64, vp, vp, vp, P(NcsnWeights), i32, f32, vp,
+                                       P(NcsnSaved), vp, vp]),
     "geossl_schnet_layer_loop": (i32, [vp, i32, vp, i32, vp, vp, vp, i32, i32, i64, i32, i32, vp]),
     "geossl_schnet_layer_loop_ragged": (i32, [vp, i32, vp, vp, vp, i64, i32, i64, i32, vp]),
     "geossl_copy2": (i32, [vp, vp, i64, vp, vp, i64, vp]),
diff --git a/geossl_amd/csrc/common.h b/geossl_amd/csrc/common.h
--- a/geossl_amd/csrc/common.h
+++ b/geossl_amd/csrc/common.h
@@ -43,6 +43,7 @@
 #pragma clang fp contract(off)
   return a + b;
 }
+__device__ __forceinline__ float ncsn_z1(float puv, float emb, float wl, float b) { return add_rn(puv, fmaf(emb, wl, b)); }
 __device__ __forceinline__ float norm2_rn(float x, float y, float z) {
 #pragma clang fp contract(off)
   const float xx = x * x, yy = y * y, zz = z * z;
diff --git a/geossl_amd/csrc/ncsn_bwd.hip b/geossl_amd/csrc/ncsn_bwd.hip
--- a/geossl_amd/csrc/ncsn_bwd.hip
+++ b/geossl_amd/csrc/ncsn_bwd.hip
@@ -76,6 +76,7 @@
   float* pw2;
   float* pb2;
   float* psm;
+  const float* proj;
 };
 
 __device__ __forceinline__ float ldg_off(const float* base, uint32_t byte_off) {
@@ -100,7 +101,7 @@
 __device__ __forceinline__ float pow2(int e) { return __builtin_amdgcn_ldexpf(1.0f, e); }
 constexpr int E_NONE = -100000;
 
-template <int NW, bool ROLE_A>
+template <int NW, bool ROLE_A, bool PRE>
 __device__ __forceinline__ void ncsn_bwd_body(const NcsnFusedArgs& a, const int S, const float* __restrict__ a_h) {
   using L_t = NbLds<NW>;
   constexpr int F = L_t::F, H = L_t::H, KHS = L_t::KHS, HMB = L_t::HMB, KS = L_t::KS, NT = 128 * NW;
@@ -126,6 +127,7 @@
   float w3r[8];
   float s_w2 = 0.0f, s_w1 = 0.0f, s_b1 = 0.0f, s_g = 0.0f, s_d = 0.0f;
   float iw1 = 0.0f, ib1 = 0.0f, iw2 = 0.0f;
+  float wl1 = 0.0f, b1c = 0.0f;
   int e3;
   {
     float m3 = 0.0f;
@@ -136,6 +138,10 @@
     iw1 = a.w.in_w1[col];
     ib1 = a.w.in_b1[col];
     iw2 = a.w.in_w2[col];
+    if constexpr (PRE) {
+      wl1 = a.w.o1_w[(size_t)col * (F + 1) + F];
+      b1c = a.w.o1_b[col];
+    }
     float raw[KHS][8];
     float wm = 0.0f, csum = 0.0f;
 #pragma unroll
@@ -232,12 +238,22 @@
       }
     }
   };
-  float a1raw[16];
+  float a1raw[16], a1rv[PRE ? 16 : 1];
   auto request_a1 = [&](int tt, int k4) {
     if constexpr (ROLE_A) {
-#pragma unroll
-      for (int r = 0; r < 16; ++r)
-        a1raw[r] = ldg_off(a.sv.a1, ((uint32_t)min(TR * tt + crow4(r, k4), S - 1) * (uint32_t)F + col) * 4u);
+      if constexpr (PRE) {
+        const int4* sc = L.scal + (tt % 3) * TR;
+#pragma unroll
+        for (int r = 0; r < 16; ++r) {
+          const int4 q = sc[crow4(r, k4)];
+          a1raw[r] = ldg_off(a.proj, ((uint32_t)q.x * (uint32_t)F + col) * 4u);
+          a1rv[r] = ldg_off(a.proj, ((uint32_t)q.y * (uint32_t)F + col) * 4u);
+        }
+      } else {
+#pragma unroll
+        for (int r = 0; r < 16; ++r)
+          a1raw[r] = ldg_off(a.sv.a1, ((uint32_t)min(TR * tt + crow4(r, k4), S - 1) * (uint32_t)F + col) * 4u);
+      }
     }
   };
   f32x4 a2raw[2];
@@ -315,7 +331,7 @@
   put_scal(t_begin + 1);
   load_scal(t_begin + 2);
   if (t_begin < t_end) {
-    request_a1(t_begin, 4 * kh);
+    if constexpr (!PRE) request_a1(t_begin, 4 * kh);
     request_a2(t_begin);
   }
   __syncthreads();
@@ -339,6 +355,7 @@
     NB_MARK(1);
     const int EGt = __builtin_amdgcn_readfirstlane(L.eg[t % 3]);
     if constexpr (ROLE_A) {
+      if constexpr (PRE) request_a1(t, k4);
       put_scal(t + 2);
       const float kT = pow2(EGt + eC - 14);
       f32x16 acc0, acc1;
@@ -367,7 +384,11 @@
         float tb = 0.0f, td = 0.0f, am = 0.0f;
 #pragma unroll
         for (int r = 0; r < 16; ++r) {
-          a1raw[r] = pin(a1raw[r]);
+          if constexpr (PRE)
+            a1raw[r] = fmaxf(ncsn_z1(add_rn(pin(a1raw[r]), pin(a1rv[r])), __int_as_float(sc[crow4(r, k4)].w), wl1, b1c),
+                             0.0f);
+          else
+            a1raw[r] = pin(a1raw[r]);
           v[r] = a1raw[r] > 0.0f ? (acc0[r] + acc1[r]) * kA : 0.0f;
           tb += v[r];
           td = fmaf(v[r], __int_as_float(sc[crow4(r, k4)].w), td);
@@ -470,7 +491,7 @@
     lds_barrier();
     NB_MARK(3);
     if constexpr (ROLE_A) {
-      request_a1(t + 1, k4);
+      if constexpr (!PRE) request_a1(t + 1, k4);
       load_scal(t + 3);
       {
         const int4* sc = L.scal + (t % 3) * TR;
@@ -618,19 +639,19 @@
 
 template <int NW>
 __global__ __launch_bounds__(128 * NW) void k_ncsn_bwd_fused(NcsnFusedArgs a) {
-  if ((int)(threadIdx.x >> 6) < NW) ncsn_bwd_body<NW, true>(a, a.S, a.h);
-  else ncsn_bwd_body<NW, false>(a, a.S, a.h);
+  if ((int)(threadIdx.x >> 6) < NW) ncsn_bwd_body<NW, true, false>(a, a.S, a.h);
+  else ncsn_bwd_body<NW, false, false>(a, a.S, a.h);
 }
 struct NcsnFusedPair { NcsnFusedArgs a[2]; };
-template <int NW>
+template <int NW, bool PRE>
 __global__ __launch_bounds__(128 * NW) void k_ncsn_bwd_fused2(NcsnFusedPair pr, const int32_t* __restrict__ dyn_S,
                                                               const int32_t* __restrict__ dyn_view) {
   const NcsnFusedArgs& a = pr.a[blockIdx.y];
   const int S = dyn_count(a.S, dyn_S);
   const float* h = a.h;
   if (dyn_view != nullptr && blockIdx.y == 1) h += (size_t)(*dyn_view) * (32 * NW);
-  if ((int)(threadIdx.x >> 6) < NW) ncsn_bwd_body<NW, true>(a, S, h);
-  else ncsn_bwd_body<NW, false>(a, S, h);
+  if ((int)(threadIdx.x >> 6) < NW) ncsn_bwd_body<NW, true, PRE>(a, S, h);
+  else ncsn_bwd_body<NW, false, PRE>(a, S, h);
 }
 
 __device__ __forceinline__ void ncsn_reduce_all_block(const ReduceMulti& m, int nblk, int accumulate,
@@ -701,7 +722,7 @@
   const int nb = fused_blocks(S), H = F / 2;
   NcsnFusedArgs a;
   a.h = h; a.sei0 = sei0; a.sei1 = sei1; a.S = (int)S; a.w = *w; a.sv = *saved; a.divisor = stats_divisor;
-  a.out_scale = out_scale; a.gout = gout; a.dfeat = dfeat; a.demb = demb; a.grow = grow;
+  a.out_scale = out_scale; a.gout = gout; a.dfeat = dfeat; a.demb = demb; a.grow = grow; a.proj = nullptr;
   a.pw1 = workspace;
   a.pd1 = a.pw1 + (size_t)nb * F * F;
   a.pb1 = a.pd1 + (size_t)nb * F;
@@ -757,12 +778,15 @@
   const int nb = (fused_blocks(S) + 1) / 2, H = F / 2;
   NcsnFusedPair pr;
   NcsnFusedArgs* a = pr.a;
+  const bool pre = heads[0].proj != nullptr && heads[1].proj != nullptr;
   for (int k = 0; k < 2; ++k) {
     const GeosslNcsnHeadBwd& hd = heads[k];
     if (hd.h == nullptr || hd.dfeat == nullptr || hd.workspace == nullptr) return (int)hipErrorInvalidValue;
+    if (!pre && hd.saved.a1 == nullptr) return (int)hipErrorInvalidValue;
     NcsnFusedArgs& x = a[k];
     x.h = hd.h; x.sei0 = sei0; x.sei1 = sei1; x.S = (int)S; x.w = hd.w; x.sv = hd.saved; x.divisor = stats_divisor;
     x.out_scale = hd.out_scale; x.gout = gout; x.dfeat = hd.dfeat; x.demb = hd.demb; x.grow = hd.grow;
+    x.proj = pre ? hd.proj : nullptr;
     x.pw1 = hd.workspace;
     x.pd1 = x.pw1 + (size_t)nb * F * F;
     x.pb1 = x.pd1 + (size_t)nb * F;
@@ -770,13 +794,17 @@
     x.pb2 = x.pw2 + (size_t)nb * H * F;
     x.psm = x.pb2 + (size_t)nb * H;
   }
-#define LAUNCH2(NWV)                                                                                                \
+#define LAUNCH2(NWV, PREV)                                                                                          \
   do {                                                                                                              \
-    allow_big_lds(&k_ncsn_bwd_fused2<NWV>);                                                                         \
-    hipLaunchKernelGGL((k_ncsn_bwd_fused2<NWV>), dim3(nb, 2), dim3(128 * NWV), NbLds<NWV>::bytes(), stream, pr,         \
-                       dyn_S, dyn_view);                                                                            \
+    allow_big_lds(&k_ncsn_bwd_fused2<NWV, PREV>);                                                                   \
+    hipLaunchKernelGGL((k_ncsn_bwd_fused2<NWV, PREV>), dim3(nb, 2), dim3(128 * NWV), NbLds<NWV>::bytes(), stream,   \
+                       pr, dyn_S, dyn_view);                                                                        \
   } while (0)
-  if (F == 128) LAUNCH2(4); else if (F == 64) LAUNCH2(2); else LAUNCH2(1);
+  if (pre) {
+    if (F == 128) LAUNCH2(4, true); else if (F == 64) LAUNCH2(2, true); else LAUNCH2(1, true);
+  } else {
+    if (F == 128) LAUNCH2(4, false); else if (F == 64) LAUNCH2(2, false); else LAUNCH2(1, false);
+  }
 #undef LAUNCH2
   GEOSSL_CHECK_LAUNCH();
   ReduceMulti rm[2];
diff --git a/geossl_amd/csrc/ncsn_rows.hip b/geossl_amd/csrc/ncsn_rows.hip
--- a/geossl_amd/csrc/ncsn_rows.hip
+++ b/geossl_amd/csrc/ncsn_rows.hip
@@ -12,7 +12,105 @@
 };
 
 template <int NMB>
-__device__ __forceinline__ void ncsn_fwd_body(const float* __restrict__ h, const int64_t* __restrict__ batch,
+__device__ __forceinline__ void format_w1(u32x4* __restrict__ W1f, const float* __restrict__ o1_w, int tid, int nthr) {
+  constexpr int F = 32 * NMB, KS = F / 16;
+  for (int i = tid; i < NMB * KS * 64; i += nthr) {
+    const int ln = i & 63, ks = (i >> 6) % KS, mb = i / (64 * KS);
+    const float* row = o1_w + (size_t)(32 * mb + (ln & 31)) * (F + 1) + 16 * ks + 8 * (ln >> 5);
+    float v[8];
+#pragma unroll
+    for (int e = 0; e < 8; ++e) v[e] = row[e];
+    const Frag3 f = split8(v);
+    u32x4* dst = W1f + ((size_t)(mb * KS + ks) * 3) * 64 + ln;
+    dst[0] = f.h;
+    dst[64] = f.m;
+    dst[128] = f.l;
+  }
+}
+template <int NMB>
+__device__ __forceinline__ void project_row(const float* __restrict__ hrow, const u32x4* __restrict__ W1f, int lane,
+                                            f32x16 (&acc)[NMB]) {
+  constexpr int F = 32 * NMB, KS = F / 16;
+  const int kh = lane >> 5;
+  f32x4 gq[2][2];
+  auto gather = [&](int ks, f32x4 (&g)[2]) {
+    const float* x = hrow + 16 * ks + 8 * kh;
+    g[0] = *reinterpret_cast<const f32x4*>(x);
+    g[1] = *reinterpret_cast<const f32x4*>(x + 4);
+  };
+  gather(0, gq[0]);
+#pragma unroll
+  for (int mb = 0; mb < NMB; ++mb)
+#pragma unroll
+    for (int r = 0; r < 16; ++r) acc[mb][r] = 0.0f;
+#pragma unroll
+  for (int ks = 0; ks < KS; ++ks) {
+    if (ks + 1 < KS) gather(ks + 1, gq[(ks + 1) & 1]);
+    const f32x4(&g)[2] = gq[ks & 1];
+    const float v[8] = {g[0].x, g[0].y, g[0].z, g[0].w, g[1].x, g[1].y, g[1].z, g[1].w};
+    const Frag3 bf = split8(v);
+    Frag3 af[NMB];
+#pragma unroll
+    for (int mb = 0; mb < NMB; ++mb) {
+      const u32x4* src = W1f + ((size_t)(mb * KS + ks) * 3) * 64 + lane;
+      af[mb].h = src[0];
+      af[mb].m = src[64];
+      af[mb].l = src[128];
+    }
+#pragma unroll
+    for (int mb = 0; mb < NMB; ++mb) acc[mb] = mfma_bf16(af[mb].l, bf.h, acc[mb]);
+#pragma unroll
+    for (int mb = 0; mb < NMB; ++mb) acc[mb] = mfma_bf16(af[mb].h, bf.l, acc[mb]);
+#pragma unroll
+    for (int mb = 0; mb < NMB; ++mb) acc[mb] = mfma_bf16(af[mb].m, bf.m, acc[mb]);
+#pragma unroll
+    for (int mb = 0; mb < NMB; ++mb) acc[mb] = mfma_bf16(af[mb].m, bf.h, acc[mb]);
+#pragma unroll
+    for (int mb = 0; mb < NMB; ++mb) acc[mb] = mfma_bf16(af[mb].h, bf.m, acc[mb]);
+#pragma unroll
+    for (int mb = 0; mb < NMB; ++mb) acc[mb] = mfma_bf16(af[mb].h, bf.h, acc[mb]);
+    __builtin_amdgcn_sched_barrier(0);
+  }
+}
+
+struct NcsnProjHead {
+  const float* h;
+  const float* o1_w;
+  float* proj;
+};
+struct NcsnProjPair { NcsnProjHead a[2]; };
+template <int NMB>
+__global__ __launch_bounds__(512) void k_ncsn_proj2(NcsnProjPair pr, int N, const int32_t* __restrict__ dyn_view) {
+  constexpr int F = 32 * NMB;
+  const NcsnProjHead& a = pr.a[blockIdx.y];
+  extern __shared__ __attribute__((aligned(16))) uint8_t smem_raw[];
+  u32x4* W1f = reinterpret_cast<u32x4*>(smem_raw);
+  const int tid = threadIdx.x, lane = tid & 63, wave = tid >> 6, j = lane & 31, kh = lane >> 5;
+  const int n = dyn_count(N, dyn_view);
+  const float* h = a.h;
+  if (dyn_view != nullptr && blockIdx.y == 1) h += (size_t)(*dyn_view) * F;
+  format_w1<NMB>(W1f, a.o1_w, tid, 512);
+  __syncthreads();
+  const int nrb = (n + 31) / 32;
+  for (int rb = blockIdx.x + gridDim.x * wave; rb < nrb; rb += gridDim.x * 8) {
+    const int row = 32 * rb + j;
+    f32x16 acc[NMB];
+    project_row<NMB>(h + (size_t)min(row, n - 1) * F, W1f, lane, acc);
+    if (row < n) {
+      float* prow = a.proj + (size_t)row * F + 4 * kh;
+#pragma unroll
+      for (int mb = 0; mb < NMB; ++mb)
+#pragma unroll
+        for (int q = 0; q < 4; ++q)
+          *reinterpret_cast<f32x4*>(prow + 32 * mb + 8 * q) =
+              f32x4{acc[mb][4 * q], acc[mb][4 * q + 1], acc[mb][4 * q + 2], acc[mb][4 * q + 3]};
+    }
+  }
+}
+
+template <int NMB, bool PRE>
+__device__ __forceinline__ void ncsn_fwd_body(const float* __restrict__ h, const float* __restrict__ proj,
+                                              const int64_t* __restrict__ batch,
                                               const int64_t* __restrict__ sei0, const int64_t* __restrict__ sei1,
                                               int S, const float* __restrict__ distance,
                                               const int64_t* __restrict__ noise_level,
@@ -21,8 +119,7 @@
                                               const GeosslNcsnSaved& sv, float* __restrict__ loss_part) {
   constexpr int F = 32 * NMB, H = F / 2, HMB = (H + 31) / 32, HP = 32 * HMB, KS = F / 16;
   extern __shared__ __attribute__((aligned(16))) uint8_t smem_raw[];
-  u32x4* W1f = reinterpret_cast<u32x4*>(smem_raw);
-  u32x4* W2f = W1f + NMB * KS * 3 * 64;
+  u32x4* W2f = reinterpret_cast<u32x4*>(smem_raw);
   float* b1s = reinterpret_cast<float*>(W2f + HMB * KS * 3 * 64);
   float* wls = b1s + F;
   float* b2s = wls + F;
@@ -31,6 +128,7 @@
   float* ib1 = iw1 + F;
   float* iw2 = ib1 + F;
   float* lred = iw2 + F;
+  u32x4* W1f = reinterpret_cast<u32x4*>(lred + 8);
   const int tid = threadIdx.x, lane = tid & 63, wave = tid >> 6, j = lane & 31, kh = lane >> 5;
   const int nrb = (S + 31) / 32;
   float lsum = 0.0f;
@@ -47,21 +145,7 @@
   int rb = blockIdx.x + gridDim.x * wave;
   RowIn cur;
   if (rb < nrb) cur = load_row(rb);
-#ifdef NCSN_STAGE_UNROLL
-#pragma unroll
-#endif
-  for (int i = tid; i < NMB * KS * 64; i += 512) {
-    const int ln = i & 63, ks = (i >> 6) % KS, mb = i / (64 * KS);
-    const float* row = w.o1_w + (size_t)(32 * mb + (ln & 31)) * (F + 1) + 16 * ks + 8 * (ln >> 5);
-    float v[8];
-#pragma unroll
-    for (int e = 0; e < 8; ++e) v[e] = row[e];
-    const Frag3 f = split8(v);
-    u32x4* dst = W1f + ((size_t)(mb * KS + ks) * 3) * 64 + ln;
-    dst[0] = f.h;
-    dst[64] = f.m;
-    dst[128] = f.l;
-  }
+  if constexpr (!PRE) format_w1<NMB>(W1f, w.o1_w, tid, 512);
 #ifdef NCSN_STAGE_UNROLL
 #pragma unroll
 #endif
@@ -98,16 +182,35 @@
     const int row = 32 * rb + j;
     const bool valid = row < S;
     const RowIn in = cur;
-    f32x4 gq[2][4];
-    auto gather = [&](int ks, f32x4 (&g)[4]) {
-      const float* hu = h + (size_t)in.u * F + 16 * ks + 8 * kh;
-      const float* hv = h + (size_t)in.v * F + 16 * ks + 8 * kh;
-      g[0] = *reinterpret_cast<const f32x4*>(hu);
-      g[1] = *reinterpret_cast<const f32x4*>(hu + 4);
-      g[2] = *reinterpret_cast<const f32x4*>(hv);
-      g[3] = *reinterpret_cast<const f32x4*>(hv + 4);
-    };
-    gather(0, gq[0]);
+    f32x16 acc1[NMB];
+    if constexpr (PRE) {
+      const float* ru = proj + (size_t)in.u * F + 4 * kh;
+      const float* rv = proj + (size_t)in.v * F + 4 * kh;
+#pragma unroll
+      for (int mb = 0; mb < NMB; ++mb) {
+        f32x4 pu[4], pv[4];
+#pragma unroll
+        for (int q = 0; q < 4; ++q) {
+          pu[q] = *reinterpret_cast<const f32x4*>(ru + 32 * mb + 8 * q);
+          pv[q] = *reinterpret_cast<const f32x4*>(rv + 32 * mb + 8 * q);
+        }
+#pragma unroll
+        for (int q = 0; q < 4; ++q) {
+          acc1[mb][4 * q] = add_rn(pu[q].x, pv[q].x);
+          acc1[mb][4 * q + 1] = add_rn(pu[q].y, pv[q].y);
+          acc1[mb][4 * q + 2] = add_rn(pu[q].z, pv[q].z);
+          acc1[mb][4 * q + 3] = add_rn(pu[q].w, pv[q].w);
+        }
+      }
+    } else {
+      f32x16 au[NMB];
+      project_row<NMB>(h + (size_t)in.u * F, W1f, lane, au);
+      project_row<NMB>(h + (size_t)in.v * F, W1f, lane, acc1);
+#pragma unroll
+      for (int mb = 0; mb < NMB; ++mb)
+#pragma unroll
+        for (int r = 0; r < 16; ++r) acc1[mb][r] = add_rn(au[mb][r], acc1[mb][r]);
+    }
     if (rb + gridDim.x * 8 < nrb) cur = load_row(rb + gridDim.x * 8);
     const float pd = add_rn(in.d, mul_rn(in.eps, in.sigma));
     float e = 0.0f;
@@ -122,47 +225,18 @@
     }
     e += __shfl_xor(e, 32, 64);
     const float emb = e + ib2;
-    f32x16 acc1[NMB];
 #pragma unroll
     for (int mb = 0; mb < NMB; ++mb)
 #pragma unroll
       for (int q = 0; q < 4; ++q) {
         const f32x4 b = *reinterpret_cast<const f32x4*>(b1s + 32 * mb + 8 * q + 4 * kh);
         const f32x4 wl = *reinterpret_cast<const f32x4*>(wls + 32 * mb + 8 * q + 4 * kh);
-        acc1[mb][4 * q] = fmaf(emb, wl.x, b.x);
-        acc1[mb][4 * q + 1] = fmaf(emb, wl.y, b.y);
-        acc1[mb][4 * q + 2] = fmaf(emb, wl.z, b.z);
-        acc1[mb][4 * q + 3] = fmaf(emb, wl.w, b.w);
-      }
-#pragma unroll
-    for (int ks = 0; ks < KS; ++ks) {
-      if (ks + 1 < KS) gather(ks + 1, gq[(ks + 1) & 1]);
-      const f32x4(&g)[4] = gq[ks & 1];
-      const float v[8] = {g[0].x + g[2].x, g[0].y + g[2].y, g[0].z + g[2].z, g[0].w + g[2].w,
-                          g[1].x + g[3].x, g[1].y + g[3].y, g[1].z + g[3].z, g[1].w + g[3].w};
-      const Frag3 bf = split8(v);
-      Frag3 af[NMB];
-#pragma unroll
-      for (int mb = 0; mb < NMB; ++mb) {
-        const u32x4* src = W1f + ((size_t)(mb * KS + ks) * 3) * 64 + lane;
-        af[mb].h = src[0];
-        af[mb].m = src[64];
-        af[mb].l = src[128];
-      }
-#pragma unroll
-      for (int mb = 0; mb < NMB; ++mb) acc1[mb] = mfma_bf16(af[mb].l, bf.h, acc1[mb]);
-#pragma unroll
-      for (int mb = 0; mb < NMB; ++mb) acc1[mb] = mfma_bf16(af[mb].h, bf.l, acc1[mb]);
-#pragma unroll
-      for (int mb = 0; mb < NMB; ++mb) acc1[mb] = mfma_bf16(af[mb].m, bf.m, acc1[mb]);
-#pragma unroll
-      for (int mb = 0; mb < NMB; ++mb) acc1[mb] = mfma_bf16(af[mb].m, bf.h, acc1[mb]);
-#pragma unroll
-      for (int mb = 0; mb < NMB; ++mb) acc1[mb] = mfma_bf16(af[mb].h, bf.m, acc1[mb]);
-#pragma unroll
-      for (int mb = 0; mb < NMB; ++mb) acc1[mb] = mfma_bf16(af[mb].h, bf.h, acc1[mb]);
-      __builtin_amdgcn_sched_barrier(0);
-    }
+        acc1[mb][4 * q] = ncsn_z1(acc1[mb][4 * q], emb, wl.x, b.x);
+        acc1[mb][4 * q + 1] = ncsn_z1(acc1[mb][4 * q + 1], emb, wl.y, b.y);
+        acc1[mb][4 * q + 2] = ncsn_z1(acc1[mb][4 * q + 2], emb, wl.z, b.z);
+        acc1[mb][4 * q + 3] = ncsn_z1(acc1[mb][4 * q + 3], emb, wl.w, b.w);
+      }
+    __builtin_amdgcn_sched_barrier(0);
     Frag3 tb[KS];
     {
       float* arow = sv.a1 != nullptr ? sv.a1 + (size_t)row * F + 4 * kh : nullptr;
@@ -254,18 +328,21 @@
   }
 }
 
-template <int NMB>
-__global__ __launch_bounds__(512) void k_ncsn_fwd(const float* __restrict__ h, const int64_t* __restrict__ batch,
+template <int NMB, bool PRE>
+__global__ __launch_bounds__(512) void k_ncsn_fwd(const float* __restrict__ h, const float* __restrict__ proj,
+                                                  const int64_t* __restrict__ batch,
                                                   const int64_t* __restrict__ sei0, const int64_t* __restrict__ sei1,
                                                   int S, const float* __restrict__ distance,
                                                   const int64_t* __restrict__ noise_level,
                                                   const float* __restrict__ dist_noise, GeosslNcsnWeights w,
                                                   float anneal_power, float* __restrict__ loss_e,
                                                   GeosslNcsnSaved sv, float* __restrict__ loss_part) {
-  ncsn_fwd_body<NMB>(h, batch, sei0, sei1, S, distance, noise_level, dist_noise, w, anneal_power, loss_e, sv, loss_part);
+  ncsn_fwd_body<NMB, PRE>(h, proj, batch, sei0, sei1, S, distance, noise_level, dist_noise, w, anneal_power, loss_e, sv,
+                          loss_part);
 }
 struct NcsnFwdHead {
   const float* h;
+  const float* proj;
   const float* distance;
   const int64_t* noise_level;
   const float* dist_noise;
@@ -276,7 +353,7 @@
   float* loss_part;
 };
 struct NcsnFwdPair { NcsnFwdHead a[2]; };
-template <int NMB>
+template <int NMB, bool PRE>
 __global__ __launch_bounds__(512) void k_ncsn_fwd2(NcsnFwdPair pr, const int64_t* __restrict__ batch,
                                                    const int64_t* __restrict__ sei0, const int64_t* __restrict__ sei1,
                                                    int S, const int32_t* __restrict__ dyn_S,
@@ -284,8 +361,8 @@
   const NcsnFwdHead& a = pr.a[blockIdx.y];
   const float* h = a.h;
   if (dyn_view != nullptr && blockIdx.y == 1) h += (size_t)(*dyn_view) * (32 * NMB);
-  ncsn_fwd_body<NMB>(h, batch, sei0, sei1, dyn_count(S, dyn_S), a.distance, a.noise_level, a.dist_noise, a.w,
-                     a.anneal_power, a.loss_e, a.sv, a.loss_part);
+  ncsn_fwd_body<NMB, PRE>(h, a.proj, batch, sei0, sei1, dyn_count(S, dyn_S), a.distance, a.noise_level, a.dist_noise,
+                          a.w, a.anneal_power, a.loss_e, a.sv, a.loss_part);
 }
 
 template <int NMB>
@@ -487,31 +564,83 @@
   return nx < 256 ? nx : 256;
 }
 
-}
-
-extern "C" int64_t geossl_ddm_loss_fwd_workspace_floats(int F) { return GEOSSL_LOSS_PARTIALS; }
-
-extern "C" int geossl_ddm_loss_fwd(const float* h, const int64_t* batch, const int64_t* sei0, const int64_t* sei1,
-                                   int64_t S, const float* distance, const int64_t* noise_level,
-                                   const float* distance_noise, const GeosslNcsnWeights* w, int F, float anneal_power,
-                                   float* loss_e, const GeosslNcsnSaved* saved, float* workspace, hipStream_t stream) {
-  if (S <= 0) return 0;
-  if (F != 32 && F != 64 && F != 128) return (int)hipErrorInvalidValue;
-  GeosslNcsnSaved sv = {nullptr, nullptr, nullptr, nullptr, nullptr};
-  if (saved != nullptr) sv = *saved;
+inline size_t fwd_lds(int F, bool pre) {
   const int NMB = F / 32, H = F / 2, HMB = (H + 31) / 32, KS = F / 16;
-  const size_t lds = (size_t)(NMB + HMB) * KS * 3 * 1024 + (size_t)(5 * F + 2 * 32 * HMB + 8) * sizeof(float);
-  dim3 grid(row_blocks_grid(S));
+  return (size_t)(HMB + (pre ? 0 : NMB)) * KS * 3 * 1024 + (size_t)(5 * F + 2 * 32 * HMB + 8) * sizeof(float);
+}
+
+int launch_proj(const NcsnProjPair& pr, int nheads, int64_t N, int F, const int32_t* dyn_view, hipStream_t stream) {
+  if (N <= 0) return 0;
+  const int nrb = (int)((N + 31) / 32);
+  int nx = (nrb + 7) / 8;
+  if (nx > 256 / nheads) nx = 256 / nheads;
+  const size_t lds = (size_t)(F / 32) * (F / 16) * 3 * 1024;
+  dim3 grid(nx, nheads);
 #define LAUNCH(NMBV)                                                                                              \
   do {                                                                                                            \
-    allow_big_lds(&k_ncsn_fwd<NMBV>);                                                                             \
-    hipLaunchKernelGGL((k_ncsn_fwd<NMBV>), grid, dim3(512), lds, stream, h, batch, sei0, sei1, (int)S, distance,  \
-                       noise_level, distance_noise, *w, anneal_power, loss_e, sv, workspace);                     \
+    allow_big_lds(&k_ncsn_proj2<NMBV>);                                                                           \
+    hipLaunchKernelGGL((k_ncsn_proj2<NMBV>), grid, dim3(512), lds, stream, pr, (int)N, dyn_view);                 \
   } while (0)
   if (F == 128) LAUNCH(4); else if (F == 64) LAUNCH(2); else LAUNCH(1);
 #undef LAUNCH
   GEOSSL_CHECK_LAUNCH();
   return 0;
+}
+
+int ncsn_fwd_single(const float* h, int64_t N, float* proj, const int64_t* batch, const int64_t* sei0,
+                    const int64_t* sei1, int64_t S, const float* distance, const int64_t* noise_level,
+                    const float* distance_noise, const GeosslNcsnWeights* w, int F, float anneal_power, float* loss_e,
+                    const GeosslNcsnSaved* saved, float* workspace, hipStream_t stream) {
+  if (S <= 0) return 0;
+  if (F != 32 && F != 64 && F != 128) return (int)hipErrorInvalidValue;
+  GeosslNcsnSaved sv = {nullptr, nullptr, nullptr, nullptr, nullptr};
+  if (saved != nullptr) sv = *saved;
+  const bool pre = proj != nullptr;
+  if (pre) {
+    NcsnProjPair pr = {};
+    pr.a[0].h = h; pr.a[0].o1_w = w->o1_w; pr.a[0].proj = proj;
+    const int rc = launch_proj(pr, 1, N, F, nullptr, stream);
+    if (rc != 0) return rc;
+  }
+  const size_t lds = fwd_lds(F, pre);
+  dim3 grid(row_blocks_grid(S));
+#define LAUNCH(NMBV, PREV)                                                                                        \
+  do {                                                                                                            \
+    allow_big_lds(&k_ncsn_fwd<NMBV, PREV>);                                                                       \
+    hipLaunchKernelGGL((k_ncsn_fwd<NMBV, PREV>), grid, dim3(512), lds, stream, h, proj, batch, sei0, sei1, (int)S, \
+                       distance, noise_level, distance_noise, *w, anneal_power, loss_e, sv, workspace);           \
+  } while (0)
+  if (pre) {
+    if (F == 128) LAUNCH(4, true); else if (F == 64) LAUNCH(2, true); else LAUNCH(1, true);
+  } else {
+    if (F == 128) LAUNCH(4, false); else if (F == 64) LAUNCH(2, false); else LAUNCH(1, false);
+  }
+#undef LAUNCH
+  GEOSSL_CHECK_LAUNCH();
+  return 0;
+}
+
+}
+
+extern "C" int64_t geossl_ddm_loss_fwd_workspace_floats(int F) { return GEOSSL_LOSS_PARTIALS; }
+
+extern "C" int geossl_ddm_loss_fwd(const float* h, const int64_t* batch, const int64_t* sei0, const int64_t* sei1,
+                                   int64_t S, const float* distance, const int64_t* noise_level,
+                                   const float* distance_noise, const GeosslNcsnWeights* w, int F, float anneal_power,
+                                   float* loss_e, const GeosslNcsnSaved* saved, float* workspace, hipStream_t stream) {
+  return ncsn_fwd_single(h, 0, nullptr, batch, sei0, sei1, S, distance, noise_level, distance_noise, w, F, anneal_power,
+                         loss_e, saved, workspace, stream);
+}
+
+extern "C" int geossl_ddm_loss_fwd_proj(const float* h, int64_t N, float* proj, const int64_t* batch,
+                                        const int64_t* sei0, const int64_t* sei1, int64_t S, const float* distance,
+                                        const int64_t* noise_level, const float* distance_noise,
+                                        const GeosslNcsnWeights* w, int F, float anneal_power, float* loss_e,
+                                        const GeosslNcsnSaved* saved, float* workspace, hipStream_t stream) {
+  if (S <= 0) return 0;
+  if (proj == nullptr || N <= 0) return (int)hipErrorInvalidValue;
+  return ncsn_fwd_single(h, N, proj, batch, sei0, sei1, S, distance, noise_level, distance_noise, w, F, anneal_power,
+                         loss_e, saved, workspace, stream);
 }
 
 extern "C" int geossl_ddm_loss_fwd2(const GeosslNcsnHeadFwd* heads, const int64_t* batch, const int64_t* sei0,
@@ -529,21 +658,35 @@
   for (int k = 0; k < 2; ++k) {
     const GeosslNcsnHeadFwd& hd = heads[k];
     if (hd.h == nullptr || hd.loss_e == nullptr) return (int)hipErrorInvalidValue;
-    a[k].h = hd.h; a[k].distance = hd.distance; a[k].noise_level = hd.noise_level; a[k].dist_noise = hd.distance_noise;
+    a[k].h = hd.h; a[k].proj = hd.proj; a[k].distance = hd.distance; a[k].noise_level = hd.noise_level; a[k].dist_noise = hd.distance_noise;
     a[k].w = hd.w; a[k].sv = hd.saved; a[k].anneal_power = hd.anneal_power; a[k].loss_e = hd.loss_e;
     a[k].loss_part = hd.workspace;
   }
-  const int NMB = F / 32, H = F / 2, HMB = (H + 31) / 32, KS = F / 16;
-  const size_t lds = (size_t)(NMB + HMB) * KS * 3 * 1024 + (size_t)(5 * F + 2 * 32 * HMB + 8) * sizeof(float);
+  const bool pre = heads[0].proj != nullptr && heads[1].proj != nullptr;
+  if (pre) {
+    if (heads[0].n_atoms <= 0 || heads[1].n_atoms != heads[0].n_atoms) return (int)hipErrorInvalidValue;
+    NcsnProjPair pp;
+    for (int k = 0; k < 2; ++k) {
+      pp.a[k].h = heads[k].h; pp.a[k].o1_w = heads[k].w.o1_w; pp.a[k].proj = heads[k].proj;
+    }
+    const int rc = launch_proj(pp, 2, heads[0].n_atoms, F, dyn_view, stream);
+    if (rc != 0) return rc;
+  }
+  const size_t lds = fwd_lds(F, pre);
   dim3 grid((row_blocks_grid(S) + 1) / 2, 2);
-#define LAUNCH(NMBV)                                                                                              \
+#define LAUNCH(NMBV, PREV)                                                                                        \
   do {                                                                                                            \
-    allow_big_lds(&k_ncsn_fwd2<NMBV>);                                                                            \
-    hipLaunchKernelGGL((k_ncsn_fwd2<NMBV>), grid, dim3(512), lds, stream, pr, batch, sei0, sei1, (int)S,           \
+    allow_big_lds(&k_ncsn_fwd2<NMBV, PREV>);                                                                      \
+    hipLaunchKernelGGL((k_ncsn_fwd2<NMBV, PREV>), grid, dim3(512), lds, stream, pr, batch, sei0, sei1, (int)S,     \
                        dyn_S, dyn_view);                                                                          \
   } while (0)
-  if (F == 128) LAUNCH(4); else if (F == 64) LAUNCH(2); else LAUNCH(1);
+  if (pre) {
+    if (F == 128) LAUNCH(4, true); else if (F == 64) LAUNCH(2, true); else LAUNCH(1, true);
+  } else {
+    if (F == 128) LAUNCH(4, false); else if (F == 64) LAUNCH(2, false); else LAUNCH(1, false);
+  }
 #undef LAUNCH
+
   GEOSSL_CHECK_LAUNCH();
   return 0;
 }
diff --git a/include/geossl_hip.h b/include/geossl_hip.h
--- a/include/geossl_hip.h
+++ b/include/geossl_hip.h
@@ -225,6 +225,10 @@
                         const float* distance, const int64_t* noise_level, const float* distance_noise,
                         const GeosslNcsnWeights* w, int F, float anneal_power, float* loss_e,
                         const GeosslNcsnSaved* saved, float* workspace, hipStream_t stream);
+int geossl_ddm_loss_fwd_proj(const float* h, int64_t N, float* proj, const int64_t* batch, const int64_t* sei0,
+                             const int64_t* sei1, int64_t S, const float* distance, const int64_t* noise_level,
+                             const float* distance_noise, const GeosslNcsnWeights* w, int F, float anneal_power,
+                             float* loss_e, const GeosslNcsnSaved* saved, float* workspace, hipStream_t stream);
 int64_t geossl_loss_reduce_workspace_floats(int64_t S);
 int geossl_loss_reduce(const float* loss_e, int64_t S, const int64_t* stats_divisor, float out_scale, float* loss,
                        float* workspace, int accumulate, hipStream_t stream);
@@ -239,6 +243,8 @@
   float pad_;
   float* loss_e;
   float* workspace;
+  float* proj;
+  int64_t n_atoms;
 } GeosslNcsnHeadFwd;
 typedef struct {
   const float* h;
@@ -252,6 +258,7 @@
   GeosslNcsnGrads grads;
   float* workspace;
   float* dh;
+  const float* proj;
 } GeosslNcsnHeadBwd;
 int geossl_ddm_loss_fwd2(const GeosslNcsnHeadFwd* heads, const int64_t* batch, const int64_t* sei0, const int64_t* sei1,
                          int64_t S, int F, hipStream_t stream);
```

Result: faster. 399,700, median of 6 (+1.3%).
